# trevorcampbell/bayesian-coresets

Measured on AMD Instinct MI355X. Metric: greedy coreset iterations/sec (N=10000000, d=512), higher is better.
Workload: dtype f32 scan + f64 state

## Files before the change

bayesian-coresets_amd/csrc/api.hip:

```cpp
#include <stdio.h>
#include <string.h>
#include <algorithm>
#include <cmath>
#include "bcx_internal.h"
#include "dev_util.h"

static thread_local std::string g_create_err;
namespace {
void bounce_acquire(int device);
void bounce_release(int device);
}

extern "C" const char* bcx_version(void) { return "bcx 0.1 gfx950"; }

extern "C" const char* bcx_last_error(const bcx_solver* s) { return s ? s->err.c_str() : g_create_err.c_str(); }

template <typename T> static hipError_t dev_alloc(T** p, size_t count, bool zero = true) {
  *p = nullptr;
  if (count == 0) count = 1;
  hipError_t e = hipMalloc((void**)p, count * sizeof(T));
  if (e != hipSuccess) return e;
  if (zero) e = hipMemset(*p, 0, count * sizeof(T));
  return e;
}

static int round_up(int x, int m) { return (x + m - 1) / m * m; }

static void free_all(bcx_solver* s) {
  void* ptrs[] = {s->An, s->A64, s->norms, s->chunk_sums, s->staging, s->st, s->b, s->bn, s->xw, s->q64, s->qst,
                  s->tmp, s->partials, s->rec_local, s->act_idx, s->act_w, s->act_rows, s->act_norm, s->gram,
                  s->hinv, s->hinv_lo, s->cvec, s->plist, s->ppos, s->nn_x, s->nn_z, s->nn_wv, s->nn_tmp, s->nn_flag, s->nn_wbak, s->nn_xr, s->tr_sel, s->tr_err,
                  s->tr_status};
  for (void* p : ptrs)
    if (p) (void)hipFree(p);
  for (size_t w = 0; w < s->peer_mbox.size(); ++w)
    if (s->peer_mbox[w] && s->peer_mbox[w] != s->mbox) (void)hipIpcCloseMemHandle(s->peer_mbox[w]);
  void* xptrs[] = {s->mbox, s->peer_tab, s->xseq, s->xprobe, s->rec_gather, s->grid_counter, s->fin_part, s->gram_work, s->warm_buf,
                   s->Aq, s->scr_sb, s->scr_partials, s->scr_stat, s->A4, s->s4_sb, s->s4_list, s->s4_counts, s->s4_head};
  for (void* p : xptrs)
    if (p) (void)hipFree(p);
  for (auto& ev : s->prof_events) { (void)hipEventDestroy(ev.first); (void)hipEventDestroy(ev.second); }
}

extern "C" int bcx_create(const bcx_config* cfg, bcx_solver** out) {
  if (!cfg || !out) { g_create_err = "bcx_create: null argument"; return BCX_ERR_ARG; }
  *out = nullptr;
  if (cfg->alg < BCX_ALG_GIGA || cfg->alg > BCX_ALG_OMP || cfg->d < 1 || cfg->n_local < 0 ||
      cfg->world_size < 1 || cfg->rank < 0 || cfg->rank >= cfg->world_size ||
      (cfg->store_dtype != BCX_F32 && cfg->store_dtype != BCX_F64 && cfg->store_dtype != BCX_F16)) {
    g_create_err = "bcx_create: invalid configuration";
    return BCX_ERR_ARG;
  }
  const int maxd = BCX_MAX_D;
  if (cfg->d > maxd) { g_create_err = "bcx_create: d exceeds the supported row length (" + std::to_string(maxd) + ")"; return BCX_ERR_ARG; }
  if (cfg->n_local >= (int64_t)0x7fffffff) { g_create_err = "bcx_create: n_local must be < 2^31 per shard"; return BCX_ERR_ARG; }
  if (cfg->row_offset % BCX_CHUNK_ROWS != 0) {
    g_create_err = "bcx_create: row_offset must be a multiple of the chunk size (1024 rows)";
    return BCX_ERR_ARG;
  }
  bcx_solver* s = new bcx_solver();
  s->cfg = *cfg;
  if (s->cfg.refresh_every == 0) s->cfg.refresh_every = 64;
  if (const char* e = bcx_dev_env("BCX_SCREEN8")) s->scr_enabled = atoi(e) != 0;
  if (const char* e = bcx_dev_env("BCX_SCREEN4_SEGCAP")) { const int v = atoi(e); if (v >= 1 && v <= BCX_S4_SEG_CAP) s->s4_seg_cap = v; }
  if (const char* e = bcx_dev_env("BCX_SCREEN4")) s->s4_enabled = atoi(e) != 0;
  hipError_t e = hipSetDevice(cfg->device);
  if (e != hipSuccess) { g_create_err = std::string("hipSetDevice: ") + hipGetErrorString(e); delete s; return BCX_ERR_HIP; }
  const int d = cfg->d;
  const int64_t n = cfg->n_local;
  s->elem = cfg->store_dtype == BCX_F32 ? 4 : (cfg->store_dtype == BCX_F16 ? 2 : 8);
  s->qelem = cfg->store_dtype == BCX_F64 ? 8 : 4;
  s->ld = round_up(d, 16 / s->elem);
  s->ld64 = round_up(d, 2);
  s->n_chunks = (n + BCX_CHUNK_ROWS - 1) / BCX_CHUNK_ROWS;
  bool ok = true;
  auto chk = [&](hipError_t r) { if (r != hipSuccess && ok) { ok = false; g_create_err = std::string("hipMalloc: ") + hipGetErrorString(r); } };
  chk(dev_alloc((char**)&s->An, (size_t)n * s->ld * s->elem));
  if (cfg->keep_exact_rows && cfg->store_dtype != BCX_F64) chk(dev_alloc(&s->A64, (size_t)n * s->ld64));
  chk(dev_alloc(&s->norms, (size_t)n));
  chk(dev_alloc(&s->chunk_sums, (size_t)s->n_chunks * (d + 1)));
  chk(dev_alloc(&s->st, 1));
  chk(dev_alloc(&s->b, (size_t)d));
  chk(dev_alloc(&s->bn, (size_t)d));
  chk(dev_alloc(&s->xw, (size_t)d));
  chk(dev_alloc(&s->q64, (size_t)2 * s->ld64));
  chk(dev_alloc((char**)&s->qst, (size_t)2 * s->ld * s->qelem));
  chk(dev_alloc(&s->tmp, (size_t)20 * d));
  s->n_partials = 0;
  chk(dev_alloc((char**)&s->partials, (size_t)bcx_scan_grid(s) * BCX_PARTIAL_BYTES));
  chk(dev_alloc(&s->rec_local, (size_t)(d + BCX_REC_HDR)));
  if (!ok) { free_all(s); delete s; return BCX_ERR_NOMEM; }
  bounce_acquire(cfg->device);
  *out = s;
  return BCX_OK;
}

extern "C" int bcx_destroy(bcx_solver* s) {
  if (!s) return BCX_OK;
  (void)hipSetDevice(s->cfg.device);
  (void)hipDeviceSynchronize();
  free_all(s);
  bounce_release(s->cfg.device);
  delete s;
  return BCX_OK;
}

extern "C" int bcx_set_stream(bcx_solver* s, void* hip_stream) {
  if (!s) return BCX_ERR_ARG;
  s->stream = (hipStream_t)hip_stream;
  return BCX_OK;
}

static int read_state(bcx_solver* s, DevState* h);

#include <mutex>
#include <thread>
namespace {
constexpr size_t kBounceBytes = (size_t)32 << 20;
constexpr int kMaxDevices = 64;
struct Bounce {
  std::mutex mu;
  void* buf[2] = {nullptr, nullptr};
  int users = 0;
};
Bounce g_bounce[kMaxDevices];
Bounce& bounce_of(int device) { return g_bounce[(device >= 0 && device < kMaxDevices) ? device : 0]; }
void bounce_acquire(int device) {
  Bounce& b = bounce_of(device);
  std::lock_guard<std::mutex> lock(b.mu);
  b.users += 1;
}
void bounce_release(int device) {
  Bounce& b = bounce_of(device);
  std::lock_guard<std::mutex> lock(b.mu);
  if (--b.users <= 0) {
    b.users = 0;
    for (int i = 0; i < 2; ++i)
      if (b.buf[i]) { (void)hipHostFree(b.buf[i]); b.buf[i] = nullptr; }
  }
}

void copy_rows_mt(char* dst, size_t dpitch, const char* src, size_t spitch, size_t width, int64_t rows) {
  const size_t bytes = (size_t)rows * width;
  int nt = (int)std::min<size_t>(8, bytes / ((size_t)2 << 20));
  const unsigned hw = std::thread::hardware_concurrency();
  if (hw && (unsigned)nt > hw) nt = (int)hw;
  auto work = [=](int64_t r0, int64_t r1) {
    if (dpitch == width && spitch == width) { memcpy(dst + (size_t)r0 * width, src + (size_t)r0 * width, (size_t)(r1 - r0) * width); return; }
    for (int64_t r = r0; r < r1; ++r) memcpy(dst + (size_t)r * dpitch, src + (size_t)r * spitch, width);
  };
  if (nt <= 1) { work(0, rows); return; }
  std::vector<std::thread> th;
  const int64_t per = (rows + nt - 1) / nt;
  for (int t = 1; t < nt; ++t) {
    const int64_t r0 = std::min<int64_t>(rows, t * per), r1 = std::min<int64_t>(rows, (t + 1) * per);
    if (r0 < r1) th.emplace_back(work, r0, r1);
  }
  work(0, std::min<int64_t>(rows, per));
  for (auto& t : th) t.join();
}
}

static int upload_host_rows(bcx_solver* s, void* dst_dev, size_t dpitch, const void* src, size_t spitch, size_t width,
                            int64_t rows) {
  if (rows <= 0) return BCX_OK;
  Bounce& g_b = bounce_of(s->cfg.device);
  std::lock_guard<std::mutex> lock(g_b.mu);
  for (int i = 0; i < 2; ++i)
    if (!g_b.buf[i]) BCX_HIP(hipHostMalloc(&g_b.buf[i], kBounceBytes, hipHostMallocPortable));
  if (width > kBounceBytes) { s->err = "bcx_load_rows: a row exceeds the upload buffer"; return BCX_ERR_ARG; }
  hipEvent_t done[2] = {nullptr, nullptr};
  bool busy[2] = {false, false};
  for (int i = 0; i < 2; ++i) {
    const hipError_t ee = hipEventCreateWithFlags(&done[i], hipEventDisableTiming);
    if (ee != hipSuccess) {
      if (i == 1) (void)hipEventDestroy(done[0]);
      s->err = std::string("upload: ") + hipGetErrorString(ee);
      return BCX_ERR_HIP;
    }
  }
  const int64_t rows_per = std::max<int64_t>(1, (int64_t)(kBounceBytes / width));
  int which = 0;
  int rc = BCX_OK;
  for (int64_t r = 0; r < rows && rc == BCX_OK; r += rows_per, which ^= 1) {
    const int64_t m = std::min(rows_per, rows - r);
    if (busy[which]) {
      if (hipEventSynchronize(done[which]) != hipSuccess) { s->err = "upload: event wait failed"; rc = BCX_ERR_HIP; break; }
      busy[which] = false;
    }
    copy_rows_mt((char*)g_b.buf[which], width, (const char*)src + (size_t)r * spitch, spitch, width, m);
    hipError_t e = hipMemcpy2DAsync((char*)dst_dev + (size_t)r * dpitch, dpitch, g_b.buf[which], width, width, (size_t)m,
                                    hipMemcpyHostToDevice, s->stream);
    if (e == hipSuccess) e = hipEventRecord(done[which], s->stream);
    if (e != hipSuccess) { s->err = std::string("upload: ") + hipGetErrorString(e); rc = BCX_ERR_HIP; break; }
    busy[which] = true;
  }
  for (int i = 0; i < 2; ++i) {
    if (busy[i]) (void)hipEventSynchronize(done[i]);
    (void)hipEventDestroy(done[i]);
  }
  return rc;
}


static int load_rows(bcx_solver* s, const void* src, int32_t src_is_device, int32_t src_dtype, int64_t row_begin,
                     int64_t rows, int64_t ld, int32_t flags);

extern "C" int bcx_load_rows(bcx_solver* s, const void* src, int32_t src_is_device, int32_t src_dtype,
                             int64_t row_begin, int64_t rows, int64_t ld) {
  return load_rows(s, src, src_is_device, src_dtype, row_begin, rows, ld, 0);
}

extern "C" int bcx_load_rows_flags(bcx_solver* s, const void* src, int32_t src_is_device, int32_t src_dtype,
                                   int64_t row_begin, int64_t rows, int64_t ld, int32_t flags) {
  if (flags & ~BCX_LOAD_CENTER_ROWS) { if (s) s->err = "bcx_load_rows_flags: unknown flag"; return BCX_ERR_ARG; }
  return load_rows(s, src, src_is_device, src_dtype, row_begin, rows, ld, flags);
}

static int load_rows(bcx_solver* s, const void* src, int32_t src_is_device, int32_t src_dtype, int64_t row_begin,
                     int64_t rows, int64_t ld, int32_t flags) {
  if (!s || (!src && rows > 0)) return BCX_ERR_ARG;
  const int center = (flags & BCX_LOAD_CENTER_ROWS) ? 1 : 0;
  const int d = s->cfg.d;
  if (rows == 0) return BCX_OK;
  if (row_begin < 0 || rows < 0 || row_begin + rows > s->cfg.n_local || ld < d ||
      (src_dtype != BCX_F32 && src_dtype != BCX_F64)) {
    s->err = "bcx_load_rows: bad range, leading dimension or dtype";
    return BCX_ERR_ARG;
  }
  if (row_begin % BCX_CHUNK_ROWS != 0 || (rows % BCX_CHUNK_ROWS != 0 && row_begin + rows != s->cfg.n_local)) {
    s->err = "bcx_load_rows: pieces must start and end on 1024-row chunk boundaries (except the last)";
    return BCX_ERR_ARG;
  }
  BCX_HIP(hipSetDevice(s->cfg.device));
  if (row_begin == 0) {
    if (s->finalized || s->rows_loaded > 0) {
      DevState h;
      int rc0 = read_state(s, &h);
      if (rc0 != BCX_OK) return rc0;
      h.zero_row = 0; h.k = 0; h.np = 0; h.hvalid = 1; h.omp_ill = 0; h.limit = 0; h.active = 0; h.halt = HALT_NONE;
      BCX_HIP(hipMemcpy(s->st, &h, sizeof h, hipMemcpyHostToDevice));
      s->finalized = false;
    }
    s->rows_loaded = 0;
  }
  const size_t esz = src_dtype == BCX_F64 ? 8 : 4;
  if (src_is_device) {
    int rc = bcx_launch_ingest(s, src, src_dtype, ld, row_begin, rows, center);
    if (rc != BCX_OK) return rc;
  } else if (s->A64 && src_dtype == BCX_F64) {
    double* dst = s->A64 + (size_t)row_begin * s->ld64;
    int rc = upload_host_rows(s, dst, (size_t)s->ld64 * 8, src, (size_t)ld * 8, (size_t)d * 8, rows);
    if (rc != BCX_OK) return rc;
    rc = bcx_launch_ingest(s, dst, BCX_F64, s->ld64, row_begin, rows, center);
    if (rc != BCX_OK) return rc;
  } else {
    const int64_t piece = std::max<int64_t>(BCX_CHUNK_ROWS,
                                            ((int64_t)(256u << 20) / (int64_t)(d * esz)) / BCX_CHUNK_ROWS * BCX_CHUNK_ROWS);
    const size_t need = (size_t)std::min(piece, rows) * d * esz;
    if (s->staging_bytes < need) {
      if (s->staging) BCX_HIP(hipFree(s->staging));
      s->staging = nullptr; s->staging_bytes = 0;
      BCX_HIP(hipMalloc(&s->staging, need));
      s->staging_bytes = need;
    }
    for (int64_t r = 0; r < rows; r += piece) {
      const int64_t m = std::min(piece, rows - r);
      int rc = upload_host_rows(s, s->staging, (size_t)d * esz, (const char*)src + (size_t)r * ld * esz, (size_t)ld * esz,
                                (size_t)d * esz, m);
      if (rc != BCX_OK) return rc;
      rc = bcx_launch_ingest(s, s->staging, src_dtype, d, row_begin + r, m, center);
      if (rc != BCX_OK) return rc;
      BCX_HIP(hipStreamSynchronize(s->stream));
    }
  }
  s->rows_loaded += rows;
  s->scr_valid = false;
  s->s4_valid = false;
  return BCX_OK;
}

extern "C" int bcx_chunk_sums(bcx_solver* s, const void** dev_ptr, int64_t* n_chunks, int64_t* chunk_rows) {
  if (!s) return BCX_ERR_ARG;
  if (dev_ptr) *dev_ptr = s->chunk_sums;
  if (n_chunks) *n_chunks = s->n_chunks;
  if (chunk_rows) *chunk_rows = BCX_CHUNK_ROWS;
  return BCX_OK;
}

extern "C" int bcx_export_chunk_sums(bcx_solver* s, void* dst_dev, int64_t cap_chunks) {
  if (!s || !dst_dev || cap_chunks < s->n_chunks) return BCX_ERR_ARG;
  BCX_HIP(hipMemcpyAsync(dst_dev, s->chunk_sums, (size_t)s->n_chunks * (s->cfg.d + 1) * 8, hipMemcpyDeviceToDevice,
                         s->stream));
  return BCX_OK;
}

static int read_state(bcx_solver* s, DevState* h) {
  BCX_HIP(hipStreamSynchronize(s->stream));
  BCX_HIP(hipMemcpy(h, s->st, sizeof(DevState), hipMemcpyDeviceToHost));
  return BCX_OK;
}

extern "C" int bcx_finalize(bcx_solver* s, const double* b_host, const void* gathered_sums_dev, int64_t n_gathered) {
  if (!s) return BCX_ERR_ARG;
  BCX_HIP(hipSetDevice(s->cfg.device));
  if (s->rows_loaded < s->cfg.n_local) { s->err = "bcx_finalize: not all rows were loaded"; return BCX_ERR_STATE; }
  if (b_host) BCX_HIP(hipMemcpyAsync(s->b, b_host, (size_t)s->cfg.d * 8, hipMemcpyHostToDevice, s->stream));
  int rc = bcx_launch_finalize(s, b_host != nullptr, (const double*)gathered_sums_dev, n_gathered);
  if (rc != BCX_OK) return rc;
  DevState h;
  rc = read_state(s, &h);
  if (rc != BCX_OK) return rc;
  if (h.zero_row != 0) {
    char buf[128];
    snprintf(buf, sizeof buf, "A must not have any 0 columns (local row %d has zero norm)", h.zero_row - 1);
    s->err = buf;
    return BCX_ERR_ZERO_ROW;
  }
  if (s->cfg.alg == BCX_ALG_GIGA && h.bnorm == 0.0) { s->err = "norm of b must be > 0"; return BCX_ERR_ZERO_B; }
  s->finalized = true;
  return BCX_OK;
}

template <typename T> static int grow(bcx_solver* s, T** p, size_t old_count, size_t new_count) {
  T* q = nullptr;
  BCX_HIP(dev_alloc(&q, new_count));
  if (*p && old_count) BCX_HIP(hipMemcpy(q, *p, old_count * sizeof(T), hipMemcpyDeviceToDevice));
  if (*p) BCX_HIP(hipFree(*p));
  *p = q;
  return BCX_OK;
}

static int ensure_slots(bcx_solver* s, int64_t need) {
  if (need <= s->cap) return BCX_OK;
  int64_t ncap = std::max<int64_t>(need, std::max<int64_t>(256, s->cap * 2));
  const size_t d = (size_t)s->cfg.d;
  int rc;
  if ((rc = grow(s, &s->act_idx, (size_t)s->cap, (size_t)ncap))) return rc;
  if ((rc = grow(s, &s->act_w, (size_t)s->cap, (size_t)ncap))) return rc;
  if ((rc = grow(s, &s->act_norm, (size_t)s->cap, (size_t)ncap))) return rc;
  if ((rc = grow(s, &s->act_rows, (size_t)s->cap * d, (size_t)ncap * d))) return rc;
  s->cap = ncap;
  return BCX_OK;
}

int bcx_ensure_gram(bcx_solver* s, int64_t need) {
  if (need <= s->gram_cap) return BCX_OK;
  const int64_t ncap = std::max<int64_t>((need + 63) / 64 * 64, std::max<int64_t>(256, s->gram_cap * 2));
  const size_t oc = (size_t)s->gram_cap, nc = (size_t)ncap;
  double* g2 = nullptr; double* h2 = nullptr; double* l2 = nullptr;
  BCX_HIP(dev_alloc(&g2, nc * nc));
  BCX_HIP(dev_alloc(&h2, nc * nc));
  BCX_HIP(dev_alloc(&l2, nc * nc));
  if (oc) {
    BCX_HIP(hipMemcpy2D(g2, nc * 8, s->gram, oc * 8, oc * 8, oc, hipMemcpyDeviceToDevice));
    BCX_HIP(hipMemcpy2D(h2, nc * 8, s->hinv, oc * 8, oc * 8, oc, hipMemcpyDeviceToDevice));
    BCX_HIP(hipMemcpy2D(l2, nc * 8, s->hinv_lo, oc * 8, oc * 8, oc, hipMemcpyDeviceToDevice));
    BCX_HIP(hipFree(s->gram));
    BCX_HIP(hipFree(s->hinv));
    BCX_HIP(hipFree(s->hinv_lo));
  }
  s->gram = g2; s->hinv = h2; s->hinv_lo = l2;
  int rc;
  if ((rc = grow(s, &s->cvec, oc, nc))) return rc;
  if ((rc = grow(s, &s->plist, oc, nc))) return rc;
  if ((rc = grow(s, &s->ppos, oc, nc))) return rc;
  if ((rc = grow(s, &s->nn_x, oc, nc))) return rc;
  if ((rc = grow(s, &s->nn_z, 0, nc))) return rc;
  if ((rc = grow(s, &s->nn_wv, 0, nc))) return rc;
  if ((rc = grow(s, &s->nn_tmp, 0, 16 * nc))) return rc;
  if ((rc = grow(s, &s->nn_flag, 0, nc))) return rc;
  if ((rc = grow(s, &s->nn_wbak, 0, nc))) return rc;
  if ((rc = grow(s, &s->nn_xr, 0, 2 * nc))) return rc;
  s->gram_cap = ncap;
  return BCX_OK;
}

static int ensure_trace(bcx_solver* s, int64_t need) {
  if (need <= s->trace_cap) return BCX_OK;
  int64_t ncap = std::max<int64_t>(need, 1024);
  int rc;
  if ((rc = grow(s, &s->tr_sel, 0, (size_t)ncap))) return rc;
  if ((rc = grow(s, &s->tr_err, 0, (size_t)ncap))) return rc;
  if ((rc = grow(s, &s->tr_status, 0, (size_t)ncap))) return rc;
  s->trace_cap = ncap;
  return BCX_OK;
}

extern "C" int bcx_build_begin(bcx_solver* s, int64_t itrs, double tol, int32_t* skip) {
  if (!s || !skip) return BCX_ERR_ARG;
  if (!s->finalized) { s->err = "bcx_build_begin: call bcx_finalize first"; return BCX_ERR_STATE; }
  BCX_HIP(hipSetDevice(s->cfg.device));
  *skip = 0;
  DevState h;
  int rc = read_state(s, &h);
  if (rc != BCX_OK) return rc;
  if (h.limit || s->cfg.n_global == 0 || itrs <= 0) { *skip = 1; return BCX_OK; }
  s->k_ub = h.k;
  if ((rc = ensure_slots(s, (int64_t)h.k + itrs))) return rc;
  if (s->cfg.alg == BCX_ALG_OMP) {
    if ((rc = bcx_ensure_gram(s, (int64_t)h.k + itrs))) return rc;
    if (!s->grid_counter && dev_alloc(&s->grid_counter, 32 ) != hipSuccess) { s->err = "grid counter allocation failed"; return BCX_ERR_NOMEM; }
    BCX_HIP(hipMemsetAsync(s->grid_counter, 0, 2 * sizeof(unsigned long long), s->stream));
    s->grid_epoch = 0;
    s->grid_dirty = false;
  }
  if ((rc = ensure_trace(s, itrs))) return rc;
  return bcx_launch_begin(s, itrs, tol);
}

static int prof_begin(bcx_solver* s) {
  if (!s->profile) return BCX_OK;
  s->prof_now = (s->prof_tick++ % s->prof_every) == 0;
  if (!s->prof_now) return BCX_OK;
  if (s->prof_used == s->prof_events.size()) {
    hipEvent_t a, b;
    BCX_HIP(hipEventCreate(&a));
    BCX_HIP(hipEventCreate(&b));
    s->prof_events.emplace_back(a, b);
  }
  BCX_HIP(hipEventRecord(s->prof_events[s->prof_used].first, s->stream));
  return BCX_OK;
}
static int prof_end(bcx_solver* s) {
  if (!s->profile || !s->prof_now) return BCX_OK;
  BCX_HIP(hipEventRecord(s->prof_events[s->prof_used].second, s->stream));
  s->prof_used++;
  return BCX_OK;
}

static int step_scan(bcx_solver* s, void* send_dev, int exact, bool with_tail) {
  if (!s->finalized) { s->err = "solver not finalized"; return BCX_ERR_STATE; }
  double* send = send_dev ? (double*)send_dev : s->rec_local;
  int rc;
  if (exact && (rc = bcx_launch_resume_exact(s))) return rc;
  if ((rc = prof_begin(s))) return rc;
  if ((rc = bcx_launch_scan(s, exact))) return rc;
  if ((rc = prof_end(s))) return rc;
  if (with_tail) return bcx_launch_tail(s, exact);
  return bcx_launch_resolve(s, send, exact);
}

static int front_scan(bcx_solver* s, int exact, bool tier, bool four) {
  int rc;
  if (exact && (rc = bcx_launch_resume_exact(s))) return rc;
  if ((rc = prof_begin(s))) return rc;
  if ((rc = (tier && !exact) ? (four ? bcx_launch_screen4(s) : bcx_launch_screen(s)) : bcx_launch_scan(s, exact))) return rc;
  return prof_end(s);
}

extern "C" int bcx_step_scan(bcx_solver* s, void* send_dev) { if (s) s->scr_batch = false; return s ? step_scan(s, send_dev, 0, false) : BCX_ERR_ARG; }
extern "C" int bcx_step_scan_exact(bcx_solver* s, void* send_dev) { if (s) s->scr_batch = false; return s ? step_scan(s, send_dev, 1, false) : BCX_ERR_ARG; }

extern "C" int bcx_step_apply(bcx_solver* s, const void* recv_dev) {
  if (!s) return BCX_ERR_ARG;
  return bcx_launch_apply(s, recv_dev ? (const double*)recv_dev : s->rec_local);
}

static int enqueue_one(bcx_solver* s, int exact, bool tier, bool four = false) {
  if (!s->finalized) { s->err = "solver not finalized"; return BCX_ERR_STATE; }
  int rc;
  if (s->cfg.world_size != 1) {
    if (!s->exchange_ready) {
      s->err = "bcx_build_enqueue on a row shard needs bcx_exchange_attach (or drive bcx_step_scan / bcx_step_apply)";
      return BCX_ERR_ARG;
    }
    if ((rc = front_scan(s, exact, tier, false))) return rc;
    return bcx_launch_tail_exchange(s, exact);
  }
  if ((rc = front_scan(s, exact, tier, four))) return rc;
  if (s->cfg.alg == BCX_ALG_OMP) {
    rc = bcx_launch_omp_fused(s, exact);
    if (rc != 1) return rc;
    if ((rc = bcx_launch_resolve(s, s->rec_local, exact))) return rc;
    return bcx_launch_apply(s, s->rec_local);
  }
  return bcx_launch_tail(s, exact);
}

static int enqueue_many(bcx_solver* s, int64_t itrs) {
  int rc = bcx_screen_build(s);
  if (rc != BCX_OK) return rc;
  const bool tier = bcx_screen_on(s) && s->scr_valid;
  if (tier && (rc = bcx_screen4_build(s))) return rc;
  const bool tier4 = tier && bcx_screen4_on(s) && s->s4_valid;
  s->scr_batch = false;
  for (int64_t i = 0; i < itrs; ++i) {
    s->scr_batch = tier;
    const bool four = tier4 && s->s4_warm == 0;
    rc = enqueue_one(s, 0, tier, four);
    if (rc != BCX_OK) return rc;
    if (tier && s->s4_warm > 0) s->s4_warm -= 1;
  }
  return BCX_OK;
}

extern "C" int bcx_build_enqueue(bcx_solver* s, int64_t itrs) {
  if (!s) return BCX_ERR_ARG;
  if (!s->finalized) { s->err = "solver not finalized"; return BCX_ERR_STATE; }
  return enqueue_many(s, itrs);
}

extern "C" int bcx_build_enqueue_exact(bcx_solver* s) {
  if (!s) return BCX_ERR_ARG;
  if (!s->finalized) { s->err = "solver not finalized"; return BCX_ERR_STATE; }
  s->scr_batch = false;
  return enqueue_one(s, 1, false);
}

static int mailbox_alloc(bcx_solver* s) {
  if (s->mbox) return BCX_OK;
  const int world = s->cfg.world_size;
  const size_t bytes = bcx_mailbox_slot_offset(world) + 2 * (size_t)world * (s->cfg.d + BCX_REC_HDR) * sizeof(double);
  hipError_t e = hipExtMallocWithFlags(&s->mbox, bytes, hipDeviceMallocFinegrained);
  if (e != hipSuccess) {
    (void)hipGetLastError();
    s->mbox = nullptr;
    s->err = std::string("peer mailbox: fine-grained allocation failed: ") + hipGetErrorString(e);
    return BCX_ERR_HIP;
  }
  s->mbox_bytes = bytes;
  BCX_HIP(hipMemset(s->mbox, 0, bytes));
  BCX_HIP(hipDeviceSynchronize());
  return BCX_OK;
}

extern "C" int bcx_exchange_export(bcx_solver* s, void* handle_out, int32_t handle_bytes) {
  if (!s || !handle_out) return BCX_ERR_ARG;
  if (handle_bytes < (int32_t)sizeof(hipIpcMemHandle_t)) { s->err = "bcx_exchange_export: handle buffer too small"; return BCX_ERR_ARG; }
  if ((size_t)s->cfg.d * sizeof(double) > 144 * 1024) {
    s->err = "peer mailbox: rows of more than 18432 values exchange their records through the all-gather";
    return BCX_ERR_ARG;
  }
  BCX_HIP(hipSetDevice(s->cfg.device));
  int rc = mailbox_alloc(s);
  if (rc != BCX_OK) return rc;
  hipIpcMemHandle_t h;
  BCX_HIP(hipIpcGetMemHandle(&h, s->mbox));
  memset(handle_out, 0, handle_bytes);
  memcpy(handle_out, &h, sizeof(h));
  return BCX_OK;
}

extern "C" int bcx_exchange_attach(bcx_solver* s, const void* handles, int32_t handle_bytes, double timeout_s) {
  if (!s || !handles) return BCX_ERR_ARG;
  if (s->exchange_ready) return BCX_OK;
  if (!s->mbox) { s->err = "bcx_exchange_attach: call bcx_exchange_export first"; return BCX_ERR_STATE; }
  if (handle_bytes < (int32_t)sizeof(hipIpcMemHandle_t)) return BCX_ERR_ARG;
  BCX_HIP(hipSetDevice(s->cfg.device));
  const int world = s->cfg.world_size;
  if (world > BCX_APPLY_THREADS) { s->err = "peer mailbox supports at most 256 shards"; return BCX_ERR_ARG; }
  s->peer_mbox.assign(world, nullptr);
  for (int w = 0; w < world; ++w) {
    if (w == s->cfg.rank) { s->peer_mbox[w] = s->mbox; continue; }
    hipIpcMemHandle_t h;
    memcpy(&h, (const char*)handles + (size_t)w * handle_bytes, sizeof(h));
    hipError_t e = hipIpcOpenMemHandle(&s->peer_mbox[w], h, hipIpcMemLazyEnablePeerAccess);
    if (e != hipSuccess) {
      (void)hipGetLastError();
      s->peer_mbox[w] = nullptr;
      s->err = "peer mailbox: cannot map shard " + std::to_string(w) + ": " + hipGetErrorString(e);
      for (int v = 0; v < w; ++v)
        if (v != s->cfg.rank && s->peer_mbox[v]) { (void)hipIpcCloseMemHandle(s->peer_mbox[v]); s->peer_mbox[v] = nullptr; }
      s->peer_mbox.clear();
      return BCX_ERR_HIP;
    }
  }
  hipError_t e;
  if ((e = dev_alloc(&s->peer_tab, (size_t)world)) != hipSuccess || (e = dev_alloc(&s->xseq, 8)) != hipSuccess ||
      (e = dev_alloc(&s->xprobe, 1)) != hipSuccess ||
      (e = dev_alloc(&s->rec_gather, (size_t)world * (s->cfg.d + BCX_REC_HDR))) != hipSuccess) {
    s->err = std::string("peer mailbox: ") + hipGetErrorString(e);
    return BCX_ERR_NOMEM;
  }
  BCX_HIP(hipMemcpy(s->peer_tab, s->peer_mbox.data(), (size_t)world * sizeof(void*), hipMemcpyHostToDevice));
  if (timeout_s > 0.0) s->exchange_timeout_s = timeout_s;
  s->exchange_ready = true;
  return BCX_OK;
}

extern "C" int bcx_exchange_probe(bcx_solver* s, int32_t* result) {
  if (!s || !result) return BCX_ERR_ARG;
  if (!s->exchange_ready) { s->err = "bcx_exchange_probe: no peer mailbox attached"; return BCX_ERR_STATE; }
  BCX_HIP(hipSetDevice(s->cfg.device));
  int rc = bcx_launch_exchange_probe(s);
  if (rc != BCX_OK) return rc;
  BCX_HIP(hipStreamSynchronize(s->stream));
  BCX_HIP(hipMemcpy(result, s->xprobe, sizeof(int32_t), hipMemcpyDeviceToHost));
  return BCX_OK;
}

extern "C" int bcx_exchange_set_timeout(bcx_solver* s, double timeout_s) {
  if (!s || !(timeout_s > 0.0)) return BCX_ERR_ARG;
  s->exchange_timeout_s = timeout_s;
  return BCX_OK;
}

extern "C" int bcx_exchange_stats(bcx_solver* s, int64_t* n, double* wait_us_mean, double* wait_us_max, double* total_us_mean,
                                  double* total_us_max, int32_t reset) {
  if (!s) return BCX_ERR_ARG;
  unsigned long long h[5] = {0, 0, 0, 0, 0};
  if (s->xseq) {
    BCX_HIP(hipSetDevice(s->cfg.device));
    BCX_HIP(hipStreamSynchronize(s->stream));
    BCX_HIP(hipMemcpy(h, s->xseq + 1, sizeof h, hipMemcpyDeviceToHost));
    if (reset) BCX_HIP(hipMemset(s->xseq + 1, 0, sizeof h));
  }
  const double per = h[0] ? 1.0 / (double)h[0] : 0.0, us = 1.0 / 100.0;
  if (n) *n = (int64_t)h[0];
  if (wait_us_mean) *wait_us_mean = (double)h[1] * per * us;
  if (wait_us_max) *wait_us_max = (double)h[2] * us;
  if (total_us_mean) *total_us_mean = (double)h[3] * per * us;
  if (total_us_max) *total_us_max = (double)h[4] * us;
  return BCX_OK;
}

extern "C" int bcx_exchange_disable(bcx_solver* s) {
  if (!s) return BCX_ERR_ARG;
  s->exchange_ready = false;
  return BCX_OK;
}

extern "C" int bcx_build_poll(bcx_solver* s, int64_t* n_done, int32_t* need_exact, int32_t* limit) {
  if (!s) return BCX_ERR_ARG;
  DevState h;
  int rc = read_state(s, &h);
  if (rc != BCX_OK) return rc;
  while (h.halt == HALT_NEED_EXACT && s->scr_batch && s->scr_stat) {
    unsigned long long st8[SCR_WORDS];
    BCX_HIP(hipMemcpy(st8, s->scr_stat, sizeof st8, hipMemcpyDeviceToHost));
    if (!st8[SCR_ARMED]) break;
    if (st8[SCR4_LAST] != 0 && st8[SCR4_LAST] == st8[SCR_ITERS]) {
      s->s4_halts += 1;
      for (int i = 3; i > 0; --i) s->s4_ovf_at[i] = s->s4_ovf_at[i - 1];
      s->s4_ovf_at[0] = st8[SCR4_ITERS];
      s->s4_redos += 1;
      if (s->s4_halts >= 4 && s->s4_ovf_at[0] - s->s4_ovf_at[3] < 256 && !s->s4_dropped) { s->s4_dropped = 1; s->s4_drops += 1; }
    } else {
      s->scr_halts += 1;
      for (int i = 3; i > 0; --i) s->scr_ovf_at[i] = s->scr_ovf_at[i - 1];
      s->scr_ovf_at[0] = st8[SCR_ITERS];
      if (s->scr_halts >= 4 && s->scr_ovf_at[0] - s->scr_ovf_at[3] < 256) s->scr_dropped = 1;
    }
    if (s->s4_warm < 1) s->s4_warm = 1;
    if ((rc = bcx_launch_resume_store(s))) return rc;
    if ((rc = enqueue_one(s, 0, false))) return rc;
    const int64_t rest = h.itrs - h.it - 1;
    if (rest > 0 && (rc = enqueue_many(s, rest))) return rc;
    else if (rest <= 0) s->scr_batch = false;
    if ((rc = read_state(s, &h))) return rc;
  }
  if (h.halt == HALT_GRID_TIMEOUT) { s->err = "OMP step: grid barrier timed out"; return BCX_ERR_STATE; }
  if (h.halt == HALT_EXCHANGE_TIMEOUT) {
    unsigned long long late[2] = {0, 0};
    std::string who;
    if (s->xseq && hipMemcpy(late, s->xseq + 6, sizeof late, hipMemcpyDeviceToHost) == hipSuccess) {
      for (int r = 0; r < s->cfg.world_size && r < 64; ++r)
        if (late[0] >> r & 1ull) who += (who.empty() ? "" : ", ") + std::to_string(r);
      (void)hipMemset(s->xseq + 6, 0, sizeof late);
    } else (void)hipGetLastError();
    s->err = "peer mailbox: rank " + std::to_string(s->cfg.rank) + " got no record from rank(s) " + (who.empty() ? "?" : who) +
             " within " + std::to_string(s->exchange_timeout_s) + " s (exchange #" + std::to_string(late[1]) + ")";
    return BCX_ERR_EXCHANGE;
  }
  if (n_done) *n_done = h.it;
  if (need_exact) *need_exact = (h.halt == HALT_NEED_EXACT);
  if (limit) *limit = h.limit;
  if (s->profile) {
    const bool on8 = bcx_screen_on(s) && s->scr_valid;
    const double min_ms = (double)s->cfg.n_local * s->cfg.d * (on8 ? ((bcx_screen4_on(s) && s->s4_valid) ? 0.5 : 1.0) : (double)s->elem) / 12.0e9;
    for (size_t i = 0; i < s->prof_used; ++i) {
      float ms = 0.f;
      if (hipEventElapsedTime(&ms, s->prof_events[i].first, s->prof_events[i].second) != hipSuccess) continue;
      if ((double)ms >= min_ms) { s->prof_ms += ms; s->prof_launches += 1; }
    }
    s->prof_used = 0;
  }
  return BCX_OK;
}

extern "C" int bcx_build_trace(bcx_solver* s, int64_t* sel, double* err, int32_t* status, int64_t cap, int64_t* n_out) {
  if (!s) return BCX_ERR_ARG;
  DevState h;
  int rc = read_state(s, &h);
  if (rc != BCX_OK) return rc;
  const int64_t n = std::min<int64_t>(h.it, cap);
  if (n > 0) {
    if (sel) BCX_HIP(hipMemcpy(sel, s->tr_sel, (size_t)n * 8, hipMemcpyDeviceToHost));
    if (err) BCX_HIP(hipMemcpy(err, s->tr_err, (size_t)n * 8, hipMemcpyDeviceToHost));
    if (status) BCX_HIP(hipMemcpy(status, s->tr_status, (size_t)n * 4, hipMemcpyDeviceToHost));
  }
  if (n_out) *n_out = n;
  return BCX_OK;
}

extern "C" int bcx_active_count(bcx_solver* s, int64_t* k) {
  if (!s || !k) return BCX_ERR_ARG;
  DevState h;
  int rc = read_state(s, &h);
  if (rc != BCX_OK) return rc;
  *k = h.k;
  return BCX_OK;
}

extern "C" int bcx_get_weights(bcx_solver* s, int64_t* idx, double* w, int64_t cap, int64_t* k) {
  if (!s || !k) return BCX_ERR_ARG;
  DevState h;
  int rc = read_state(s, &h);
  if (rc != BCX_OK) return rc;
  const int64_t n = std::min<int64_t>(h.k, cap);
  if (n > 0) {
    if (idx) BCX_HIP(hipMemcpy(idx, s->act_idx, (size_t)n * 8, hipMemcpyDeviceToHost));
    if (w) BCX_HIP(hipMemcpy(w, s->act_w, (size_t)n * 8, hipMemcpyDeviceToHost));
  }
  *k = h.k;
  return BCX_OK;
}

extern "C" int bcx_error(bcx_solver* s, double* err) {
  if (!s || !err) return BCX_ERR_ARG;
  if (!s->finalized) { s->err = "solver not finalized"; return BCX_ERR_STATE; }
  int rc = bcx_launch_error_refresh(s);
  if (rc != BCX_OK) return rc;
  DevState h;
  if ((rc = read_state(s, &h))) return rc;
  *err = h.err;
  return BCX_OK;
}

extern "C" int bcx_reached_numeric_limit(bcx_solver* s, int32_t* limit) {
  if (!s || !limit) return BCX_ERR_ARG;
  DevState h;
  int rc = read_state(s, &h);
  if (rc != BCX_OK) return rc;
  *limit = h.limit;
  return BCX_OK;
}

extern "C" int bcx_reset(bcx_solver* s) {
  if (!s) return BCX_ERR_ARG;
  if (!s->finalized) return BCX_OK;
  DevState h;
  int rc = read_state(s, &h);
  if (rc != BCX_OK) return rc;
  h.k = 0; h.np = 0; h.hvalid = 1; h.omp_ill = 0; h.limit = 0; h.retried = 0; h.active = 0; h.halt = HALT_NONE; h.since_refresh = 0; h.exact_mode = 0;
  h.err = h.bnorm; h.nw = 1.0; h.it = 0; h.itrs = 0;
  BCX_HIP(hipMemcpy(s->st, &h, sizeof h, hipMemcpyHostToDevice));
  BCX_HIP(hipMemset(s->xw, 0, (size_t)s->cfg.d * 8));
  if (s->scr_dropped == 1) s->scr_dropped = 0;
  s->scr_halts = 0;
  for (int i = 0; i < 4; ++i) s->scr_ovf_at[i] = 0;
  if (s->s4_dropped == 1) s->s4_dropped = 0;
  s->s4_halts = 0;
  for (int i = 0; i < 4; ++i) s->s4_ovf_at[i] = 0;
  s->s4_warm = 2;
  return bcx_launch_error_refresh(s);
}

extern "C" int bcx_set_check_monotone(bcx_solver* s, int32_t on) {
  if (!s) return BCX_ERR_ARG;
  BCX_HIP(hipSetDevice(s->cfg.device));
  DevState h;
  int rc = read_state(s, &h);
  if (rc != BCX_OK) return rc;
  h.no_monotone = on ? 0 : 1;
  BCX_HIP(hipMemcpy(s->st, &h, sizeof h, hipMemcpyHostToDevice));
  return BCX_OK;
}

extern "C" int bcx_optimize(bcx_solver* s, double tol, int32_t* accepted) {
  if (!s || !accepted) return BCX_ERR_ARG;
  if (!s->finalized) { s->err = "solver not finalized"; return BCX_ERR_STATE; }
  DevState h;
  int rc = read_state(s, &h);
  if (rc != BCX_OK) return rc;
  if ((rc = ensure_slots(s, std::max<int64_t>(h.k, 1)))) return rc;
  if ((rc = bcx_ensure_gram(s, std::max<int64_t>(h.k, 1)))) return rc;
  if ((rc = bcx_launch_optimize(s, tol))) return rc;
  DevState h2;
  if ((rc = read_state(s, &h2))) return rc;
  if (h2.halt == HALT_GRID_TIMEOUT) { s->err = "optimize: grid barrier timed out"; return BCX_ERR_STATE; }
  *accepted = h2.limit ? 0 : 1;
  return BCX_OK;
}

extern "C" int bcx_get_vector(bcx_solver* s, int32_t which, double* out) {
  if (!s || !out) return BCX_ERR_ARG;
  const double* src = nullptr;
  switch (which) {
    case 0: src = s->b; break;
    case 1: src = s->xw; break;
    case 2: src = s->q64; break;
    case 3: src = s->q64 + s->ld64; break;
    default: return BCX_ERR_ARG;
  }
  BCX_HIP(hipStreamSynchronize(s->stream));
  BCX_HIP(hipMemcpy(out, src, (size_t)s->cfg.d * 8, hipMemcpyDeviceToHost));
  return BCX_OK;
}

extern "C" int bcx_get_norms(bcx_solver* s, int64_t begin, int64_t count, double* out) {
  if (!s || !out || begin < 0 || begin + count > s->cfg.n_local) return BCX_ERR_ARG;
  BCX_HIP(hipStreamSynchronize(s->stream));
  BCX_HIP(hipMemcpy(out, s->norms + begin, (size_t)count * 8, hipMemcpyDeviceToHost));
  return BCX_OK;
}

extern "C" int bcx_get_stored_rows(bcx_solver* s, int64_t begin, int64_t count, void* out, int32_t* ld_out) {
  if (!s || begin < 0 || count < 0 || begin + count > s->cfg.n_local) return BCX_ERR_ARG;
  if (ld_out) *ld_out = s->ld;
  if (count == 0) return BCX_OK;
  if (!out) return BCX_ERR_ARG;
  BCX_HIP(hipSetDevice(s->cfg.device));
  BCX_HIP(hipStreamSynchronize(s->stream));
  BCX_HIP(hipMemcpy(out, (const char*)s->An + (size_t)begin * s->ld * s->elem, (size_t)count * s->ld * s->elem, hipMemcpyDeviceToHost));
  return BCX_OK;
}

extern "C" int bcx_time_scan(bcx_solver* s, int32_t reps, int32_t exact, double* ms_per_launch, double* bytes_per_launch) {
  if (!s || reps < 1) return BCX_ERR_ARG;
  if (!s->finalized) { s->err = "solver not finalized"; return BCX_ERR_STATE; }
  BCX_HIP(hipSetDevice(s->cfg.device));
  DevState h;
  int rc = read_state(s, &h);
  if (rc != BCX_OK) return rc;
  DevState forced = h;
  forced.active = 1;
  BCX_HIP(hipMemcpy(s->st, &forced, sizeof forced, hipMemcpyHostToDevice));
  hipEvent_t e0, e1;
  BCX_HIP(hipEventCreate(&e0));
  BCX_HIP(hipEventCreate(&e1));
  for (int i = 0; i < 3 && rc == BCX_OK; ++i) rc = bcx_launch_scan(s, exact);
  if (rc == BCX_OK) (void)hipEventRecord(e0, s->stream);
  for (int i = 0; i < reps && rc == BCX_OK; ++i) rc = bcx_launch_scan(s, exact);
  if (rc != BCX_OK) {
    (void)hipEventDestroy(e0); (void)hipEventDestroy(e1);
    (void)hipMemcpy(s->st, &h, sizeof h, hipMemcpyHostToDevice);
    return rc;
  }
  BCX_HIP(hipEventRecord(e1, s->stream));
  BCX_HIP(hipEventSynchronize(e1));
  float ms = 0.f;
  BCX_HIP(hipEventElapsedTime(&ms, e0, e1));
  BCX_HIP(hipEventDestroy(e0));
  BCX_HIP(hipEventDestroy(e1));
  BCX_HIP(hipMemcpy(s->st, &h, sizeof h, hipMemcpyHostToDevice));
  if (ms_per_launch) *ms_per_launch = (double)ms / reps;
  const bool raw64 = exact && s->cfg.store_dtype != BCX_F64 && s->A64;
  if (bytes_per_launch) *bytes_per_launch = (double)s->cfg.n_local * s->cfg.d * (raw64 ? 8.0 : (double)s->elem);
  return BCX_OK;
}

extern "C" int bcx_argmax_correlation(bcx_solver* s, const double* query_host, int64_t* idx, double* score) {
  if (!s || !query_host || !idx || !score) return BCX_ERR_ARG;
  if (!s->finalized) { s->err = "solver not finalized"; return BCX_ERR_STATE; }
  if (s->cfg.alg == BCX_ALG_GIGA) { s->err = "bcx_argmax_correlation needs a single-query solver (FW/OMP)"; return BCX_ERR_ARG; }
  BCX_HIP(hipSetDevice(s->cfg.device));
  const int d = s->cfg.d;
  DevState h;
  int rc = read_state(s, &h);
  if (rc != BCX_OK) return rc;
  std::vector<double> q64((size_t)s->ld64, 0.0);
  double qmax = 0.0;
  for (int j = 0; j < d; ++j) { q64[j] = query_host[j]; qmax = std::fmax(qmax, std::fabs(query_host[j])); }
  const bool scalable = qmax > 0.0 && qmax < INFINITY;
  const int E0 = scalable ? std::ilogb(qmax) : 0;
  double qn = 0.0;
  for (int j = 0; j < d; ++j) { const double t = std::ldexp(query_host[j], -E0); qn += t * t; }
  qn = std::sqrt(qn);
  int E = 0;
  BCX_HIP(hipMemcpy(s->q64, q64.data(), (size_t)s->ld64 * 8, hipMemcpyHostToDevice));
  if (s->cfg.store_dtype == BCX_F64) {
    std::vector<double> qs((size_t)s->ld, 0.0);
    for (int j = 0; j < d; ++j) qs[j] = query_host[j];
    BCX_HIP(hipMemcpy(s->qst, qs.data(), (size_t)s->ld * 8, hipMemcpyHostToDevice));
    qn = std::ldexp(qn, E0);
  } else {
    const int E1 = (scalable && qn > 0.0 && qn < INFINITY) ? std::ilogb(qn) : 0;
    E = E0 + E1;
    std::vector<float> qs((size_t)s->ld, 0.f);
    for (int j = 0; j < d; ++j) qs[j] = (float)std::ldexp(query_host[j], -E);
    BCX_HIP(hipMemcpy(s->qst, qs.data(), (size_t)s->ld * 4, hipMemcpyHostToDevice));
    qn = std::ldexp(qn, -E1);
  }
  DevState forced = h;
  forced.active = 1; forced.exact_mode = 0; forced.qscale = qn; forced.qexp = E;
  double rec[BCX_REC_HDR];
  for (int attempt = 0; attempt < 2; ++attempt) {
    forced.exact_mode = attempt;
    BCX_HIP(hipMemcpy(s->st, &forced, sizeof forced, hipMemcpyHostToDevice));
    if ((rc = bcx_launch_scan(s, attempt))) return rc;
    if ((rc = bcx_launch_resolve(s, s->rec_local, attempt))) return rc;
    BCX_HIP(hipStreamSynchronize(s->stream));
    BCX_HIP(hipMemcpy(rec, s->rec_local, sizeof rec, hipMemcpyDeviceToHost));
    if (rec[3] != BCX_REC_OVERFLOW) break;
  }
  BCX_HIP(hipMemcpy(s->st, &h, sizeof h, hipMemcpyHostToDevice));
  if (rec[3] != BCX_REC_VALID) { s->err = "no rows to scan"; return BCX_ERR_STATE; }
  *idx = (int64_t)rec[1];
  *score = rec[0];
  return BCX_OK;
}

extern "C" int bcx_stats(bcx_solver* s, int64_t* exact_fallbacks, int64_t* candidates, int64_t* resolves) {
  if (!s) return BCX_ERR_ARG;
  DevState h;
  int rc = read_state(s, &h);
  if (rc != BCX_OK) return rc;
  if (exact_fallbacks) *exact_fallbacks = h.n_exact;
  if (candidates) *candidates = h.n_cand;
  if (resolves) *resolves = h.n_resolved;
  return BCX_OK;
}

extern "C" int bcx_screen_stats(bcx_solver* s, int64_t* out8) {
  if (!s || !out8) return BCX_ERR_ARG;
  unsigned long long st8[SCR_WORDS] = {0, 0, 0, 0, 0, 0, 0, 0};
  if (s->scr_stat) {
    BCX_HIP(hipSetDevice(s->cfg.device));
    BCX_HIP(hipStreamSynchronize(s->stream));
    BCX_HIP(hipMemcpy(st8, s->scr_stat, sizeof st8, hipMemcpyDeviceToHost));
  }
  const bool possible = s->scr_enabled && s->cfg.store_dtype != BCX_F64 && s->cfg.d <= 4096 && s->cfg.n_local > 0;
  out8[0] = bcx_screen_on(s) ? 1 : 0;
  out8[1] = (int64_t)st8[SCR_ITERS];
  out8[2] = (int64_t)st8[SCR_SURVIVORS];
  out8[3] = (int64_t)st8[SCR_OVERFLOWS];
  out8[4] = (int64_t)st8[SCR_REDOS];
  out8[5] = !possible ? 3 : s->scr_dropped;
  out8[6] = s->Aq ? (int64_t)s->scr_cap_rows * (s->ld8 + 8) + (int64_t)BCX_MAX_PARTIALS * BCX_PARTIAL_BYTES + SCR_WORDS * 8 : 0;
  out8[7] = (int64_t)(s->scr_build_ms * 1e3f);
  return BCX_OK;
}

extern "C" int bcx_screen4_stats(bcx_solver* s, int64_t* out8) {
  if (!s || !out8) return BCX_ERR_ARG;
  unsigned long long st8[SCR_WORDS];
  for (auto& w : st8) w = 0;
  if (s->scr_stat) {
    BCX_HIP(hipSetDevice(s->cfg.device));
    BCX_HIP(hipStreamSynchronize(s->stream));
    BCX_HIP(hipMemcpy(st8, s->scr_stat, sizeof st8, hipMemcpyDeviceToHost));
  }
  const bool possible = s->s4_enabled && s->scr_enabled && s->cfg.store_dtype != BCX_F64 && s->cfg.d <= 4096 && s->cfg.n_local > 0 &&
                        s->cfg.alg != BCX_ALG_GIGA && s->cfg.world_size == 1;
  if (st8[SCR4_PENDING] && s->s4_counts && s->s4_n_seg > 0) {
    std::vector<int32_t> cnt((size_t)s->s4_n_seg);
    BCX_HIP(hipMemcpy(cnt.data(), s->s4_counts, cnt.size() * 4, hipMemcpyDeviceToHost));
    for (int32_t c : cnt) { st8[SCR4_LISTED] += (unsigned long long)std::min<int32_t>(c, s->s4_seg_cap); st8[SCR4_OVERFLOWS] += c > s->s4_seg_cap; }
  }
  out8[0] = bcx_screen4_on(s) ? 1 : 0;
  out8[1] = (int64_t)st8[SCR4_ITERS];
  out8[2] = (int64_t)st8[SCR4_LISTED];
  out8[3] = (int64_t)st8[SCR4_OVERFLOWS];
  out8[4] = s->s4_redos;
  out8[5] = !possible ? 3 : s->s4_dropped;
  out8[6] = s->A4 ? (int64_t)s->s4_cap_rows * (s->ld4 + 8) + (int64_t)BCX_MAX_PARTIALS * (BCX_S4_SEG_CAP + 1) * 4 : 0;
  out8[7] = s->s4_drops;
  return BCX_OK;
}

extern "C" int bcx_screen_read(bcx_solver* s, int64_t begin, int64_t count, void* codes, float* scales, float* bounds, int32_t* ld8_out) {
  if (!s || begin < 0 || count < 0 || begin + count > s->cfg.n_local) return BCX_ERR_ARG;
  if (!s->finalized) { s->err = "solver not finalized"; return BCX_ERR_STATE; }
  BCX_HIP(hipSetDevice(s->cfg.device));
  int rc = bcx_screen_build(s);
  if (rc != BCX_OK) return rc;
  if (!bcx_screen_on(s) || !s->scr_valid) { s->err = "bcx_screen_read: the 8-bit tier is not in use"; return BCX_ERR_STATE; }
  BCX_HIP(hipStreamSynchronize(s->stream));
  if (ld8_out) *ld8_out = s->ld8;
  if (count == 0) return BCX_OK;
  if (codes) BCX_HIP(hipMemcpy(codes, (const char*)s->Aq + (size_t)begin * s->ld8, (size_t)count * s->ld8, hipMemcpyDeviceToHost));
  std::vector<float> sb((size_t)count * 2);
  BCX_HIP(hipMemcpy(sb.data(), (const char*)s->scr_sb + (size_t)begin * 8, (size_t)count * 8, hipMemcpyDeviceToHost));
  for (int64_t i = 0; i < count; ++i) {
    if (scales) scales[i] = sb[2 * i];
    if (bounds) bounds[i] = sb[2 * i + 1];
  }
  return BCX_OK;
}

extern "C" int bcx_omp_stats(bcx_solver* s, int64_t* out4) {
  if (!s || !out4) return BCX_ERR_ARG;
  DevState h;
  int rc = read_state(s, &h);
  if (rc != BCX_OK) return rc;
  for (int i = 0; i < 4; ++i) out4[i] = h.n_omp[i];
  out4[2] += s->opt_fallbacks;
  return BCX_OK;
}

extern "C" int bcx_profile_scan(bcx_solver* s, int32_t on) {
  if (!s) return BCX_ERR_ARG;
  s->profile = on != 0;
  s->prof_every = on > 1 ? on : 1;
  s->prof_tick = 0;
  s->prof_ms = 0.0;
  s->prof_launches = 0;
  s->prof_used = 0;
  return BCX_OK;
}

extern "C" int bcx_profile_read(bcx_solver* s, double* scan_ms_total, int64_t* scan_launches) {
  if (!s) return BCX_ERR_ARG;
  if (scan_ms_total) *scan_ms_total = s->prof_ms;
  if (scan_launches) *scan_launches = s->prof_launches;
  return BCX_OK;
}

extern "C" int bcx_debug_stamps(bcx_solver* s, long long* out32) {
  DevState h;
  int rc = read_state(s, &h);
  if (rc != BCX_OK) return rc;
  for (int i = 0; i < 32; ++i) out32[i] = h.dbg_t[i];
  return BCX_OK;
}

extern "C" int bcx_debug_wbak(bcx_solver* s, double* out, int32_t count) {
  if (!s || !s->nn_wbak || count > s->gram_cap) return BCX_ERR_ARG;
  BCX_HIP(hipDeviceSynchronize());
  BCX_HIP(hipMemcpy(out, s->nn_wbak, (size_t)count * sizeof(double), hipMemcpyDeviceToHost));
  return BCX_OK;
}
```

bayesian-coresets_amd/csrc/bcx_internal.h:

```cpp
#pragma once
#include <hip/hip_runtime.h>
#include <stdint.h>
#include <string>
#include <utility>
#include <vector>
#include "../../include/bcx.h"

#define BCX_CHUNK_ROWS 1024
#define BCX_MAX_CAND 64
#define BCX_REC_HDR 4
#define BCX_REC_VALID 1.0
#define BCX_REC_OVERFLOW 2.0
#define BCX_MAX_D BCX_MAX_ROW_LENGTH
#define BCX_SCAN_THREADS 256
#define BCX_APPLY_THREADS 256

enum { HALT_NONE = 0, HALT_DONE = 1, HALT_LIMIT = 2, HALT_NEED_EXACT = 3, HALT_EXCHANGE_TIMEOUT = 4, HALT_GRID_TIMEOUT = 5 };
enum { OMP_IDLE = 0, OMP_DONE = 1, OMP_FAST_TRY = 2, OMP_FAST_ACCEPT = 3, OMP_GENERAL = 4,
       OMP_OPT_FALLBACK = 5 };

struct PartialView {
  double *U1, *U2, *U3, *L;
  int32_t *i1, *i2;
};
#define BCX_PARTIAL_BYTES 40
#define BCX_MAX_PARTIALS 2048
#define BCX_SCREEN_MAX_SURV 256
enum { SCR_ARMED = 0,
       SCR_ITERS = 1,
       SCR_SURVIVORS = 2,
       SCR_OVERFLOWS = 3,
       SCR_REDOS = 4,
       SCR4_ITERS = 5,
       SCR4_LISTED = 6,
       SCR4_OVERFLOWS = 7,
       SCR4_LAST = 8,
       SCR4_PENDING = 9,
       SCR_WORDS = 10 };
#define BCX_S4_SEG_CAP 1024
#define BCX_S4_SENTINELS 64
static inline __host__ __device__ PartialView partial_view(void* base, int n) {
  PartialView v;
  v.U1 = (double*)base; v.U2 = v.U1 + n; v.U3 = v.U2 + n; v.L = v.U3 + n;
  v.i1 = (int32_t*)(v.L + n); v.i2 = v.i1 + n;
  return v;
}

struct Mailbox {
  void* const* peers;
  unsigned long long* seq;
  int32_t* probe;
  unsigned long long* stat;
  int world, rank, recw;
  unsigned off_slots;
  long long timeout_ticks;
};

static inline unsigned bcx_mailbox_slot_offset(int world) { return (unsigned)((2u * world * 8u + 255u) / 256u * 256u); }

struct DevState {
  int64_t itrs;
  int64_t it;
  int32_t active;
  int32_t halt;
  int32_t retried;
  int32_t limit;
  int32_t k;
  int32_t since_refresh;
  int32_t exact_mode;
  int32_t zero_row;
  int32_t no_monotone;
  int32_t np;
  int32_t hvalid;
  int32_t hlo_valid;
  int32_t omp_mode;
  int32_t omp_slot, omp_fresh, omp_checked, omp_p;
  int32_t omp_ill;
  int64_t omp_f;
  double omp_nf, omp_gff, omp_cf, omp_t, omp_inv;
  double tol;
  double err;
  double nw;
  double bnorm;
  double sigma;
  int64_t n_exact;
  int64_t n_cand;
  int64_t n_resolved;
  int64_t n_omp[4];
  double qscale;
  int32_t qexp;
  int32_t qexp_pad;
  long long dbg_t[32];
};

struct bcx_solver {
  bcx_config cfg;
  hipStream_t stream = nullptr;
  std::string err;
  int ld = 0;
  int elem = 4;
  int qelem = 4;
  int ld64 = 0;
  void* An = nullptr;
  double* A64 = nullptr;
  double* norms = nullptr;
  double* chunk_sums = nullptr;
  int64_t n_chunks = 0;
  void* staging = nullptr;
  size_t staging_bytes = 0;
  DevState* st = nullptr;
  double* b = nullptr;
  double* bn = nullptr;
  double* xw = nullptr;
  double* q64 = nullptr;
  void* qst = nullptr;
  double* tmp = nullptr;
  void* partials = nullptr;
  int n_partials = 0;
  double* rec_local = nullptr;
  double* fin_part = nullptr;
  int64_t fin_cap = 0;
  void* mbox = nullptr;
  size_t mbox_bytes = 0;
  std::vector<void*> peer_mbox;
  void** peer_tab = nullptr;
  unsigned long long* xseq = nullptr;
  int32_t* xprobe = nullptr;
  double* rec_gather = nullptr;
  bool exchange_ready = false;
  double exchange_timeout_s = 20.0;
  int64_t cap = 0;
  int64_t* act_idx = nullptr;
  double* act_w = nullptr;
  double* act_rows = nullptr;
  double* act_norm = nullptr;
  double* gram = nullptr;
  double* hinv = nullptr;
  double* hinv_lo = nullptr;
  double* cvec = nullptr;
  int32_t* plist = nullptr;
  int32_t* ppos = nullptr;
  double* nn_x = nullptr;
  double* nn_z = nullptr;
  double* nn_wv = nullptr;
  double* nn_tmp = nullptr;
  int32_t* nn_flag = nullptr;
  double* nn_wbak = nullptr;
  double* nn_xr = nullptr;
  int64_t gram_cap = 0;
  double* gram_work = nullptr;
  size_t gram_work_bytes = 0;
  void* warm_buf = nullptr;
  size_t warm_bytes = 0;
  int64_t opt_warm = 0, opt_warm_failed = 0;
  int64_t k_ub = 0;
  unsigned long long* grid_counter = nullptr;
  uint64_t grid_epoch = 0;
  int64_t opt_fallbacks = 0;
  bool grid_dirty = false;
  size_t omp_lds_allowed = 0;
  int64_t trace_cap = 0;
  int64_t* tr_sel = nullptr;
  double* tr_err = nullptr;
  int32_t* tr_status = nullptr;
  bool finalized = false;
  int64_t rows_loaded = 0;
  void* Aq = nullptr;
  void* scr_sb = nullptr;
  void* scr_partials = nullptr;
  unsigned long long* scr_stat = nullptr;
  int ld8 = 0;
  int64_t scr_cap_rows = 0;
  bool scr_enabled = true;
  int scr_dropped = 0;
  bool scr_valid = false;
  bool scr_batch = false;
  float scr_build_ms = 0.f;
  uint64_t scr_ovf_at[4] = {0, 0, 0, 0};
  int64_t scr_halts = 0;
  int scr_n_in = 0;
  void* A4 = nullptr;
  void* s4_sb = nullptr;
  void* s4_list = nullptr;
  void* s4_counts = nullptr;
  void* s4_head = nullptr;
  int ld4 = 0;
  int s4_n_seg = 0;
  int s4_seg_cap = BCX_S4_SEG_CAP;
  int64_t s4_cap_rows = 0;
  bool s4_enabled = true;
  int s4_dropped = 0;
  bool s4_valid = false;
  int s4_warm = 2;
  uint64_t s4_ovf_at[4] = {0, 0, 0, 0};
  int64_t s4_halts = 0;
  int64_t s4_redos = 0, s4_drops = 0;
  bool profile = false;
  bool prof_now = false;
  int prof_every = 1;
  int64_t prof_tick = 0;
  double prof_ms = 0.0;
  int64_t prof_launches = 0;
  std::vector<std::pair<hipEvent_t, hipEvent_t>> prof_events;
  size_t prof_used = 0;
};

int bcx_launch_ingest(bcx_solver* s, const void* src, int src_dtype, int64_t ld_src, int64_t row_begin, int64_t rows,
                      int center);
int bcx_launch_finalize(bcx_solver* s, int have_b, const double* gathered, int64_t n_gathered);
int bcx_launch_scan(bcx_solver* s, int exact);
int bcx_launch_resolve(bcx_solver* s, double* send_dev, int exact);
int bcx_launch_begin(bcx_solver* s, int64_t itrs, double tol);
int bcx_launch_apply(bcx_solver* s, const double* recv_dev);
int bcx_launch_tail(bcx_solver* s, int exact);
int bcx_launch_omp_fused(bcx_solver* s, int exact);
int bcx_launch_tail_exchange(bcx_solver* s, int exact);
int bcx_launch_exchange_probe(bcx_solver* s);
Mailbox bcx_mailbox(const bcx_solver* s);
int bcx_launch_resume_exact(bcx_solver* s);
int bcx_launch_error_refresh(bcx_solver* s);
int bcx_launch_optimize(bcx_solver* s, double tol);
int64_t bcx_gram_rows_scratch_bytes(int k, int d);
int bcx_gram_rows(hipStream_t st, const double* rows, int k, int d, int64_t ld, double* G, int64_t ldg, double* work);
unsigned long long bcx_gram_sk_epoch_now();
int bcx_gram_sk_timed_out(hipStream_t st, const double* work, unsigned long long since);
int bcx_scan_grid(const bcx_solver* s);
bool bcx_screen_on(const bcx_solver* s);
int bcx_screen_build(bcx_solver* s);
int bcx_launch_screen(bcx_solver* s);
int bcx_launch_resume_store(bcx_solver* s);
int bcx_launch_refine(bcx_solver* s, int n_in);
bool bcx_screen4_on(const bcx_solver* s);
int bcx_screen4_build(bcx_solver* s);
int bcx_launch_screen4(bcx_solver* s);
void bcx_project_set_error(const std::string& msg);
const double* proj_tables();

#ifdef BCX_TIMING
#define BCX_STAMP(st, i) do { if (threadIdx.x == 0) (st)->dbg_t[i] = wall_clock64(); } while (0)
#else
#define BCX_STAMP(st, i) do {} while (0)
#endif

#define BCX_HIP(call)                                                        \
  do {                                                                       \
    hipError_t _e = (call);                                                  \
    if (_e != hipSuccess) {                                                  \
      s->err = std::string(#call) + ": " + hipGetErrorString(_e);            \
      return BCX_ERR_HIP;                                                    \
    }                                                                        \
  } while (0)
```

bayesian-coresets_amd/csrc/screen4.hip:

```cpp
#include <float.h>
#include "screen_core.h"

#define BCX_S4_CLIP 0.8
#define BCX_S4_QMAX 1911.0
#define BCX_THRESH_THREADS 1024

struct Front4Head { float Lg, qstep, eA, eB; };

template <int CTRL> __device__ __forceinline__ int dpp_mov_i(int v) { return __builtin_amdgcn_update_dpp(0, v, CTRL, 0xf, 0xf, false); }
template <int G> __device__ __forceinline__ int group_allsum_i32(int v) {
  if (G >= 2) v += dpp_mov_i<0xB1>(v);
  if (G >= 4) v += dpp_mov_i<0x4E>(v);
  if (G >= 8) v += dpp_mov_i<0x141>(v);
  if (G >= 16) v += dpp_mov_i<0x140>(v);
  if (G >= 32) { const v2u r = __builtin_amdgcn_permlane16_swap((unsigned)v, (unsigned)v, false, false); const unsigned x = r.x, y = r.y; v = (int)(x + y); }
  if (G >= 64) { const v2u r = __builtin_amdgcn_permlane32_swap((unsigned)v, (unsigned)v, false, false); const unsigned x = r.x, y = r.y; v = (int)(x + y); }
  return v;
}

static __device__ __forceinline__ float round_up_f32(double v) {
  float f = (float)v;
  if ((double)f < v) f = nextafterf(f, INFINITY);
  return f;
}

struct Thresh4Args {
  PartialView in;
  int n_in;
  const unsigned char* Aq;
  const float2* sb;
  const float* q;
  const DevState* st;
  unsigned long long* stat;
  unsigned* head;
  const int* counts;
  int n_seg;
  int seg_cap;
  int64_t n;
  int ld8, d, nw4;
  float kacc, err_coef;
};

__global__ __launch_bounds__(BCX_THRESH_THREADS) void thresh4_kernel(Thresh4Args a) {
  if (!a.st->active) return;
  __shared__ double scratch[BCX_SCRATCH];
  const int tid = threadIdx.x, lane = tid & 63, wave = tid >> 6;
  constexpr int NW = BCX_THRESH_THREADS / 64;
  constexpr int PT = 2 * BCX_MAX_PARTIALS / BCX_THRESH_THREADS;
  double cu[PT];
  int ci[PT];
#pragma unroll
  for (int t = 0; t < PT; ++t) {
    const int c = wave + NW * (lane + 64 * t);
    const int p = c >> 1;
    const bool ok = p < a.n_in;
    const double u = ok ? ((c & 1) ? a.in.U2[p] : a.in.U1[p]) : -INFINITY;
    const int i = ok ? ((c & 1) ? a.in.i2[p] : a.in.i1[p]) : -1;
    const bool use = u > -INFINITY && i >= 0 && (int64_t)i < a.n;
    cu[t] = use ? u : -INFINITY; ci[t] = use ? i : -1;
  }
  double m = 0.0;
  for (int j = tid; j < a.d; j += BCX_THRESH_THREADS) {
    const double v = fabs((double)a.q[j]);
    m = fmax(m, v == v ? v : INFINITY);
  }
  m = block_allmax(m, scratch);
  float step = (float)(m / BCX_S4_QMAX);
  const bool qok = m < INFINITY && step >= FLT_MIN;
  if (!qok) step = 0.0f;
  constexpr int SPW = BCX_S4_SENTINELS / NW;
  int rows[SPW];
#pragma unroll
  for (int r = 0; r < SPW; ++r) {
    double best = -INFINITY;
    int bt = -1, bi = -1;
#pragma unroll
    for (int t = 0; t < PT; ++t) if (cu[t] > best) { best = cu[t]; bt = t; bi = ci[t]; }
    const double wm = wave_allmax(best);
    const unsigned long long bal = __ballot(bt >= 0 && best == wm);
    const int src = bal ? __ffsll((long long)bal) - 1 : 0;
    const int row = __shfl(bi, src, BCX_WAVE);
    rows[r] = bal ? row : -1;
#pragma unroll
    for (int t = 0; t < PT; ++t) if (bal && lane == src && t == bt) cu[t] = -INFINITY;
  }
  double acc[SPW];
#pragma unroll
  for (int r = 0; r < SPW; ++r) acc[r] = 0.0;
  const int nw8 = a.ld8 / 4;
  const unsigned* A8 = (const unsigned*)a.Aq;
  for (int w = lane; w < nw8; w += 64) {
    unsigned cw[SPW];
#pragma unroll
    for (int r = 0; r < SPW; ++r) cw[r] = A8[(int64_t)(rows[r] < 0 ? 0 : rows[r]) * nw8 + w];
    double qv[4];
#pragma unroll
    for (int k = 0; k < 4; ++k) { const int j = 4 * w + k; const float t = a.q[j < a.d ? j : 0]; qv[k] = j < a.d ? (double)t : 0.0; }
#pragma unroll
    for (int r = 0; r < SPW; ++r)
#pragma unroll
      for (int k = 0; k < 4; ++k) acc[r] = fma((double)((int)((cw[r] >> (8 * k)) & 0xffu) - 128), qv[k], acc[r]);
  }
  double err2[3] = {0.0, 0.0, 0.0};
  if (a.stat[SCR4_PENDING])
    for (int p = tid; p < a.n_seg; p += BCX_THRESH_THREADS) {
      const int c = a.counts[p];
      err2[1] += (double)(c > a.seg_cap ? a.seg_cap : c);
      err2[2] += c > a.seg_cap ? 1.0 : 0.0;
    }
  for (int w = tid; w < a.nw4; w += BCX_THRESH_THREADS) {
    unsigned p0 = 0, p1 = 0, p2 = 0;
#pragma unroll
    for (int k = 0; k < 8; ++k) {
      const int j = 8 * w + k;
      int x = 0;
      if (j < a.d && qok) {
        const double v = (double)a.q[j];
        double c = rint(v / (double)step);
        c = c > BCX_S4_QMAX ? BCX_S4_QMAX : (c < -BCX_S4_QMAX ? -BCX_S4_QMAX : c);
        x = (int)c;
        const double r = v - c * (double)step;
        err2[0] = fma(r, r, err2[0]);
      }
      const int l = ((x + 8) & 15) - 8;
      const int x1 = (x - l) >> 4;
      const int h1 = ((x1 + 8) & 15) - 8;
      const int h2 = (x1 - h1) >> 4;
      p0 |= (unsigned)(l & 15) << (4 * k); p1 |= (unsigned)(h1 & 15) << (4 * k); p2 |= (unsigned)(h2 & 15) << (4 * k);
    }
    a.head[4 + w] = p0; a.head[4 + a.nw4 + w] = p1; a.head[4 + 2 * a.nw4 + w] = p2;
  }
  block_allsum<3>(err2, scratch);
  const double qerr = sqrt(err2[0]) * (1.0 + 9.5367431640625e-07);
  const float qscale = (float)a.st->qscale;
  float lmax = -INFINITY;
#pragma unroll
  for (int r = 0; r < SPW; ++r) {
    const double tot = wave_allsum(acc[r]);
    const float2 sb = a.sb[rows[r] < 0 ? 0 : rows[r]];
    const float s0 = (float)((double)sb.x * tot);
    float U, L;
    screen_interval(s0, sb.x, sb.y, a.kacc, a.err_coef, qscale, U, L);
    if (rows[r] >= 0) lmax = fmaxf(lmax, L);
  }
  const double lg = block_allmax((double)lmax, scratch);
  if (tid == 0) {
    const double qs = (double)qscale;
    Front4Head h;
    h.Lg = qok ? (float)lg : -INFINITY;
    h.qstep = step;
    h.eA = round_up_f32((qs * 1.000002 + qerr) * 1.000004);
    h.eB = round_up_f32(((double)a.err_coef * qs + 1.001 * qerr) * 1.000004 + 1e-37);
    *(Front4Head*)a.head = h;
    a.stat[SCR4_LAST] = a.stat[SCR_ITERS] + 1ull;
    a.stat[SCR4_ITERS] += 1ull;
    a.stat[SCR4_LISTED] += (unsigned long long)err2[1];
    a.stat[SCR4_OVERFLOWS] += (unsigned long long)err2[2];
    a.stat[SCR4_PENDING] = 1ull;
  }
}

struct Front4Args {
  const uint4* A4;
  const float2* sb;
  const unsigned* head;
  const DevState* st;
  int* list;
  int* counts;
  int64_t n;
  int ldv, nw4, seg_cap;
};

template <int G, int CH, int UR>
__global__ __launch_bounds__(BCX_SCAN_THREADS) void front4_kernel(Front4Args a) {
  if (!a.st->active) return;
  constexpr int RPW = 64 / G;
  constexpr int WAVES = BCX_SCREEN_WAVES;
  constexpr int RPB = WAVES * RPW * UR;
  const int lane = threadIdx.x & 63, wave = threadIdx.x >> 6;
  const int sub = lane % G, rsub = lane / G;
  const Front4Head h = *(const Front4Head*)a.head;
  const unsigned* planes = a.head + 4;
  int qp[CH][4][3];
  int voff[CH];
#pragma unroll
  for (int c = 0; c < CH; ++c) {
    const int v = c * G + sub;
    const bool ok = v < a.ldv;
    voff[c] = ok ? v : 0;
#pragma unroll
    for (int k = 0; k < 4; ++k)
#pragma unroll
      for (int p = 0; p < 3; ++p) {
        const unsigned w = planes[p * a.nw4 + 4 * voff[c] + k];
        qp[c][k][p] = ok ? (int)w : 0;
      }
  }
  const int b = blockIdx.x * WAVES + wave;
  int* seg = a.list + (size_t)b * BCX_S4_SEG_CAP;
  int cnt = 0;
  const int64_t n = a.n;
  const int64_t stride = (int64_t)gridDim.x * RPB;
  for (int64_t r0 = (int64_t)blockIdx.x * RPB; r0 < n; r0 += stride) {
    uint4 x[UR][CH];
    float2 sbv[UR];
#pragma unroll
    for (int u = 0; u < UR; ++u) {
      const int64_t rw = r0 + (int64_t)(u * WAVES + wave) * RPW + rsub;
      const int64_t rc = rw < n ? rw : n - 1;
      const uint4* p = a.A4 + rc * a.ldv;
#pragma unroll
      for (int c = 0; c < CH; ++c) x[u][c] = stream_load(p + voff[c]);
      sbv[u] = a.sb[rc];
    }
    __builtin_amdgcn_sched_barrier(0);
#pragma unroll
    for (int u = 0; u < UR; ++u) {
      int a0 = 0, a1 = 0, a2 = 0;
#pragma unroll
      for (int c = 0; c < CH; ++c) {
        const unsigned xs[4] = {x[u][c].x, x[u][c].y, x[u][c].z, x[u][c].w};
#pragma unroll
        for (int k = 0; k < 4; ++k) {
          const int cw = (int)(xs[k] ^ 0x88888888u);
          a0 = __builtin_amdgcn_sdot8(cw, qp[c][k][0], a0, false);
          a1 = __builtin_amdgcn_sdot8(cw, qp[c][k][1], a1, false);
          a2 = __builtin_amdgcn_sdot8(cw, qp[c][k][2], a2, false);
        }
      }
      const int tot = group_allsum_i32<G>((a2 * 16 + a1) * 16 + a0);
      const float s4 = (sbv[u].x * h.qstep) * (float)tot;
      const float e4 = fmaf(sbv[u].y, h.eA, h.eB) + fabsf(s4) * 5e-7f;
      const float U4 = s4 + e4;
      const int64_t rw = r0 + (int64_t)(u * WAVES + wave) * RPW + rsub;
      const bool want = rw < n && sub == 0 && !(U4 < h.Lg);
      const unsigned long long bal = __ballot(want);
      if (bal) {
        const int pos = cnt + (int)__builtin_amdgcn_mbcnt_hi((unsigned)(bal >> 32), __builtin_amdgcn_mbcnt_lo((unsigned)bal, 0u));
        if (want && pos < a.seg_cap) seg[pos] = (int)rw;
        cnt += __popcll(bal);
      }
    }
  }
  if (lane == 0) a.counts[b] = cnt;
}

struct Second8Args {
  const uint4* Aq;
  const float2* sb;
  const float* q;
  const DevState* st;
  const int* list;
  const int* counts;
  PartialView out;
  int ldv, d, seg_cap;
  float kacc, err_coef;
};

template <int G, int CH, int UR>
__global__ __launch_bounds__(BCX_SCAN_THREADS) void second8_kernel(Second8Args a) {
  if (!a.st->active) return;
  constexpr int RPW = 64 / G;
  constexpr int WAVES = BCX_SCREEN_WAVES;
  const int lane = threadIdx.x & 63, wave = threadIdx.x >> 6;
  const int sub = lane % G, rsub = lane / G;
  const int b = blockIdx.x * WAVES + wave;
  const int cnt = __builtin_amdgcn_readfirstlane(a.counts[b]);
  const bool ovf = cnt > a.seg_cap;

  Track<float> tr;
  tr.U1 = tr.U2 = tr.U3 = tr.L = -INFINITY;
  tr.i1 = tr.i2 = 0x7fffffff;
  if (!ovf && cnt > 0) {
    Q16 q0[CH];
    int voff[CH];
    float qs0 = 0.0f;
#pragma unroll
    for (int c = 0; c < CH; ++c) {
      const int v = c * G + sub;
      const bool ok = v < a.ldv;
      voff[c] = ok ? v : 0;
      q0[c] = load_q16(a.q, v, a.d, ok, qs0);
    }
    const float off0 = -128.0f * qs0;
    const float qscale = (float)a.st->qscale;
    const int* seg = a.list + (size_t)b * BCX_S4_SEG_CAP;
    int nxt[UR];
#pragma unroll
    for (int u = 0; u < UR; ++u) { const int kk = u * RPW + rsub; nxt[u] = kk < cnt ? seg[kk] : -1; }
    for (int k0 = 0; k0 < cnt; k0 += RPW * UR) {
      int row[UR];
      uint4 x[UR][CH];
      float2 sbv[UR];
#pragma unroll
      for (int u = 0; u < UR; ++u) row[u] = nxt[u];
#pragma unroll
      for (int u = 0; u < UR; ++u) { const int kk = k0 + RPW * UR + u * RPW + rsub; nxt[u] = kk < cnt ? seg[kk] : -1; }
#pragma unroll
      for (int u = 0; u < UR; ++u) {
        const int64_t rc = row[u] < 0 ? 0 : row[u];
        const uint4* p = a.Aq + rc * a.ldv;
#pragma unroll
        for (int c = 0; c < CH; ++c) x[u][c] = stream_load(p + voff[c]);
        sbv[u] = a.sb[rc];
      }
      __builtin_amdgcn_sched_barrier(0);
#pragma unroll
      for (int u = 0; u < UR; ++u) {
        float t0 = off0;
#pragma unroll
        for (int c = 0; c < CH; ++c) t0 = dot16(x[u][c], q0[c], t0);
        float s0 = group_allsum<float, G>(t0);
        s0 *= sbv[u].x;
        float U, L;
        screen_interval(s0, sbv[u].x, sbv[u].y, a.kacc, a.err_coef, qscale, U, L);
        if (row[u] < 0) { U = -INFINITY; L = -INFINITY; }
        track_update<float>(tr, U, L, row[u] < 0 ? 0x7fffffff : row[u]);
      }
    }
#pragma unroll
    for (int off = G; off < 64; off <<= 1) tr = merge<float>(tr, shfl_track<float>(tr, off));
  }
  if (lane == 0) {
    if (ovf) {
      tr.U1 = tr.U2 = tr.L = -INFINITY; tr.U3 = INFINITY; tr.i1 = tr.i2 = 0x7fffffff;
    }
    a.out.U1[b] = (double)tr.U1; a.out.U2[b] = (double)tr.U2; a.out.U3[b] = (double)tr.U3; a.out.L[b] = (double)tr.L;
    a.out.i1[b] = tr.i1; a.out.i2[b] = tr.i2;
  }
}

template <bool F16>
__global__ __launch_bounds__(256) void quantise4_kernel(const void* An, int ld, int d, int nw4, int64_t n, unsigned* A4, float2* sb) {
  const int lane = threadIdx.x & 63;
  const int64_t row = (int64_t)blockIdx.x * 4 + (threadIdx.x >> 6);
  if (row >= n) return;
  auto elem = [&](int j) -> float {
    if (F16) return __half2float(((const __half*)An)[row * (int64_t)ld + j]);
    return ((const float*)An)[row * (int64_t)ld + j];
  };
  float m = 0.0f;
  for (int j = lane; j < d; j += 64) m = fmaxf(m, fabsf(elem(j)));
  m = (float)wave_allmax((double)m);
  float sc = (float)((double)m * BCX_S4_CLIP / 7.0);
  if (!(sc >= FLT_MIN)) sc = FLT_MIN;
  const double dsc = (double)sc;
  double r2 = 0.0;
  for (int w = lane; w < nw4; w += 64) {
    unsigned word = 0;
#pragma unroll
    for (int k = 0; k < 8; ++k) {
      const int j = 8 * w + k;
      int code = 0;
      if (j < d) {
        const double v = (double)elem(j);
        double c = rint(v / dsc);
        c = c > 7.0 ? 7.0 : (c < -7.0 ? -7.0 : c);
        if (c != c) c = 0.0;
        code = (int)c;
        const double r = v - c * dsc;
        r2 = fma(r, r, r2);
      }
      word |= (unsigned)(code + 8) << (4 * k);
    }
    A4[row * (int64_t)nw4 + w] = word;
  }
  r2 = wave_allsum(r2);
  if (lane == 0) {
    const double b = sqrt(r2) * (1.0 + 9.5367431640625e-07);
    float bf = (float)b;
    if ((double)bf < b) bf = nextafterf(bf, INFINITY);
    if (!(bf == bf)) bf = INFINITY;
    sb[row] = make_float2(sc, bf);
  }
}

bool bcx_screen4_on(const bcx_solver* s) {
  return s->s4_enabled && !s->s4_dropped && bcx_screen_on(s) && s->cfg.alg != BCX_ALG_GIGA && s->cfg.world_size == 1;
}

static size_t head_bytes(int nw4) { return sizeof(Front4Head) + (size_t)3 * nw4 * 4; }

int bcx_screen4_build(bcx_solver* s) {
  if (s->s4_valid || !bcx_screen4_on(s) || !s->scr_valid) return BCX_OK;
  const int d = s->cfg.d;
  const int64_t n = s->cfg.n_local;
  s->ld4 = (d + 31) / 32 * 16;
  const int nw4 = s->ld4 / 4;
  if (s->s4_cap_rows < n || !s->A4) {
    void** all[] = {&s->A4, &s->s4_sb, &s->s4_list, &s->s4_counts, &s->s4_head};
    for (void** p : all) { if (*p) (void)hipFree(*p); *p = nullptr; }
    s->s4_cap_rows = 0;
    hipError_t e = hipMalloc(&s->A4, (size_t)n * s->ld4);
    if (e == hipSuccess) e = hipMalloc(&s->s4_sb, (size_t)n * 8);
    if (e == hipSuccess) e = hipMalloc(&s->s4_list, (size_t)BCX_MAX_PARTIALS * BCX_S4_SEG_CAP * 4);
    if (e == hipSuccess) e = hipMalloc(&s->s4_counts, (size_t)BCX_MAX_PARTIALS * 4);
    if (e == hipSuccess) e = hipMalloc(&s->s4_head, head_bytes(nw4));
    if (e != hipSuccess) {
      (void)hipGetLastError();
      for (void** p : all) { if (*p) (void)hipFree(*p); *p = nullptr; }
      s->s4_dropped = 2;
      return BCX_OK;
    }
    s->s4_cap_rows = n;
    BCX_HIP(hipMemsetAsync(s->s4_counts, 0, (size_t)BCX_MAX_PARTIALS * 4, s->stream));
    BCX_HIP(hipMemsetAsync(s->scr_stat + SCR4_PENDING, 0, sizeof(unsigned long long), s->stream));
    s->s4_n_seg = 0;
  }
  const unsigned grid = (unsigned)((n + 3) / 4);
  if (s->cfg.store_dtype == BCX_F16)
    hipLaunchKernelGGL((quantise4_kernel<true>), dim3(grid), dim3(256), 0, s->stream, s->An, s->ld, d, nw4, n, (unsigned*)s->A4, (float2*)s->s4_sb);
  else
    hipLaunchKernelGGL((quantise4_kernel<false>), dim3(grid), dim3(256), 0, s->stream, s->An, s->ld, d, nw4, n, (unsigned*)s->A4, (float2*)s->s4_sb);
  BCX_HIP(hipGetLastError());
  s->s4_valid = true;
  s->s4_warm = 2;
  return BCX_OK;
}

static int launch_front4(bcx_solver* s, const Front4Args& a, int G, int CH, int UR, int grid) {
  dim3 g(grid), b(BCX_SCAN_THREADS);
#define L(GG, CC, UU)                                                                  \
  if (G == GG && CH == CC && UR == UU) {                                               \
    hipLaunchKernelGGL((front4_kernel<GG, CC, UU>), g, b, 0, s->stream, a);            \
    return BCX_OK;                                                                     \
  }
  L(1, 1, 4) L(2, 1, 4) L(4, 1, 4) L(8, 1, 4) L(16, 1, 4) L(32, 1, 4) L(64, 1, 4) L(64, 2, 4)
  L(1, 1, 8) L(2, 1, 8) L(4, 1, 8) L(8, 1, 8) L(16, 1, 8) L(32, 1, 8) L(64, 1, 8)
#undef L
  s->err = "front4: unsupported row length";
  return BCX_ERR_ARG;
}

static int launch_second8(bcx_solver* s, const Second8Args& a, int G, int CH, int grid) {
  dim3 g(grid), b(BCX_SCAN_THREADS);
#define L(GG, CC, UU)                                                                  \
  if (G == GG && CH == CC) {                                                           \
    hipLaunchKernelGGL((second8_kernel<GG, CC, UU>), g, b, 0, s->stream, a);           \
    return BCX_OK;                                                                     \
  }
  L(1, 1, 16) L(2, 1, 16) L(4, 1, 16) L(8, 1, 16) L(16, 1, 16) L(32, 1, 16) L(64, 1, 16) L(64, 2, 8) L(64, 4, 4)
#undef L
  s->err = "second8: unsupported row length";
  return BCX_ERR_ARG;
}

int bcx_launch_screen4(bcx_solver* s) {
  const int d = s->cfg.d;
  const int64_t n = s->cfg.n_local;
  const int nw4 = s->ld4 / 4;
  ScanArgs sa;
  ScanPlan sp;
  int rc = bcx_scan_plan(s, 0, &sa, &sp);
  if (rc != BCX_OK) return rc;
  const int ldv8 = s->ld8 / 16;
  const int G8 = screen_group(ldv8), CH8 = screen_chunks(ldv8, G8);
  const float kacc = screen_kacc(G8, CH8, d);

  Thresh4Args t;
  t.in = partial_view(s->scr_partials, s->scr_n_in); t.n_in = s->scr_n_in;
  t.Aq = (const unsigned char*)s->Aq; t.sb = (const float2*)s->scr_sb; t.q = (const float*)s->qst;
  t.st = s->st; t.stat = s->scr_stat; t.head = (unsigned*)s->s4_head;
  t.n = n; t.ld8 = s->ld8; t.d = d; t.nw4 = nw4;
  t.kacc = kacc; t.err_coef = sa.err_coef;

  Front4Args f;
  f.A4 = (const uint4*)s->A4; f.sb = (const float2*)s->s4_sb; f.head = (const unsigned*)s->s4_head; f.st = s->st;
  f.list = (int*)s->s4_list; f.counts = (int*)s->s4_counts;
  f.n = n; f.ldv = s->ld4 / 16; f.nw4 = nw4;
  const int G = screen_group(f.ldv), CH = screen_chunks(f.ldv, G);
  const int ur = CH == 1 ? 8 : 4;
  const int rpb = BCX_SCREEN_WAVES * (64 / G) * ur;
  const int64_t want = (n + rpb - 1) / rpb;
  int cap = 512;
  if (cap > BCX_MAX_PARTIALS / BCX_SCREEN_WAVES) cap = BCX_MAX_PARTIALS / BCX_SCREEN_WAVES;
  const int grid = (int)(want < 1 ? 1 : (want > cap ? cap : want));
  t.counts = (const int*)s->s4_counts; t.n_seg = s->s4_n_seg; t.seg_cap = s->s4_seg_cap;
  f.seg_cap = s->s4_seg_cap;
  hipLaunchKernelGGL(thresh4_kernel, dim3(1), dim3(BCX_THRESH_THREADS), 0, s->stream, t);
  BCX_HIP(hipGetLastError());
  s->s4_n_seg = grid * BCX_SCREEN_WAVES;
  if ((rc = launch_front4(s, f, G, CH, ur, grid))) return rc;

  const int n_in = grid * BCX_SCREEN_WAVES;
  Second8Args c;
  c.Aq = (const uint4*)s->Aq; c.sb = (const float2*)s->scr_sb; c.q = (const float*)s->qst; c.st = s->st;
  c.list = (const int*)s->s4_list; c.counts = (const int*)s->s4_counts;
  c.out = partial_view(s->scr_partials, n_in);
  c.ldv = ldv8; c.d = d; c.seg_cap = s->s4_seg_cap; c.kacc = kacc; c.err_coef = sa.err_coef;
  if ((rc = launch_second8(s, c, G8, CH8, grid))) return rc;
  BCX_HIP(hipGetLastError());
  s->scr_n_in = n_in;
  return bcx_launch_refine(s, n_in);
}
```

bayesian-coresets_amd/csrc/screen8.hip:

```cpp
#include <float.h>
#include "screen_core.h"

#define BCX_REFINE_THREADS 1024

struct ScreenArgs {
  const uint4* Aq;
  const float2* sb;
  const float* q;
  const DevState* st;
  PartialView out;
  int64_t n;
  int ldv;
  int ldq;
  int d;
  float kacc;
  float err_coef;
};

template <bool DUAL, int G, int CH, int UR>
__global__ __launch_bounds__(BCX_SCAN_THREADS) void screen_kernel(ScreenArgs a) {
  if (!a.st->active) return;
  constexpr int RPW = 64 / G;
  constexpr int WAVES = BCX_SCREEN_WAVES;
  constexpr int RPB = WAVES * RPW * UR;
  constexpr bool PACK4 = G >= 4 && (UR % 4 == 0);
  constexpr int GSZ = PACK4 ? G / 4 : G;
  constexpr int NT = PACK4 ? UR / 4 : UR;
  const int lane = threadIdx.x & 63, wave = threadIdx.x >> 6;
  const int sub = lane % G, rsub = lane / G;
  int myu = 0, myrs = 0;
  if constexpr (PACK4) pack_map<G>(lane, myu, myrs);

  Q16 q0[CH], q1[CH];
  int voff[CH];
  float qs0 = 0.0f, qs1 = 0.0f;
#pragma unroll
  for (int c = 0; c < CH; ++c) {
    const int v = c * G + sub;
    const bool ok = v < a.ldv;
    voff[c] = ok ? v : 0;
    q0[c] = load_q16(a.q, v, a.d, ok, qs0);
    if (DUAL) q1[c] = load_q16(a.q + a.ldq, v, a.d, ok, qs1);
  }
  const float off0 = -128.0f * qs0, off1 = -128.0f * qs1;
  const float qscale = (float)a.st->qscale;

  Track<float> tr;
  tr.U1 = tr.U2 = tr.U3 = tr.L = -INFINITY;
  tr.i1 = tr.i2 = 0x7fffffff;

  const uint4* base = a.Aq;
  const int64_t n = a.n;
  auto row_of = [&](int64_t r0, int u) { return r0 + (int64_t)(u * WAVES + wave) * RPW + rsub; };
  auto tracked = [&](int64_t r0, int t) {
    if constexpr (PACK4) return r0 + (int64_t)((t * 4 + myu) * WAVES + wave) * RPW + myrs;
    else return row_of(r0, t);
  };
  const int64_t stride = (int64_t)gridDim.x * RPB;
  for (int64_t r0 = (int64_t)blockIdx.x * RPB; r0 < n; r0 += stride) {
    uint4 x[UR][CH];
    float2 sbv[NT];
#pragma unroll
    for (int u = 0; u < UR; ++u) {
      const int64_t rw = row_of(r0, u);
      const int64_t rc = rw < n ? rw : n - 1;
      const uint4* p = base + rc * a.ldv;
#pragma unroll
      for (int c = 0; c < CH; ++c) x[u][c] = stream_load(p + voff[c]);
    }
#pragma unroll
    for (int t = 0; t < NT; ++t) { const int64_t rw = tracked(r0, t); sbv[t] = a.sb[rw < n ? rw : n - 1]; }
    __builtin_amdgcn_sched_barrier(0);
#pragma unroll
    for (int t = 0; t < NT; ++t) {
      float s0, s1 = 0.0f;
      if constexpr (PACK4) {
        float a0[4], a1[4];
#pragma unroll
        for (int u = 0; u < 4; ++u) {
          float t0 = off0, t1 = off1;
#pragma unroll
          for (int c = 0; c < CH; ++c) {
            t0 = dot16(x[t * 4 + u][c], q0[c], t0);
            if (DUAL) t1 = dot16(x[t * 4 + u][c], q1[c], t1);
          }
          a0[u] = t0; a1[u] = t1;
        }
        s0 = reduce4_pack<G, float>(a0[0], a0[1], a0[2], a0[3]);
        if (DUAL) s1 = reduce4_pack<G, float>(a1[0], a1[1], a1[2], a1[3]);
      } else {
        float t0 = off0, t1 = off1;
#pragma unroll
        for (int c = 0; c < CH; ++c) {
          t0 = dot16(x[t][c], q0[c], t0);
          if (DUAL) t1 = dot16(x[t][c], q1[c], t1);
        }
        s0 = group_allsum<float, G>(t0);
        if (DUAL) s1 = group_allsum<float, G>(t1);
      }
      const int64_t myrow = tracked(r0, t);
      const float scale = sbv[t].x, bound = sbv[t].y;
      s0 *= scale; s1 *= scale;
      float U, L;
      if (DUAL) giga_interval(s0, s1, (fmaf(scale, a.kacc, bound) * 1.000002f + a.err_coef) * qscale, U, L);
      else screen_interval(s0, scale, bound, a.kacc, a.err_coef, qscale, U, L);
      if (!(myrow < n)) { U = -INFINITY; L = -INFINITY; }
      track_update<float>(tr, U, L, (int)myrow);
    }
  }
#pragma unroll
  for (int off = GSZ; off < 64; off <<= 1) tr = merge<float>(tr, shfl_track<float>(tr, off));
  if (lane == 0) {
    const int b = blockIdx.x * WAVES + wave;
    a.out.U1[b] = (double)tr.U1; a.out.U2[b] = (double)tr.U2; a.out.U3[b] = (double)tr.U3; a.out.L[b] = (double)tr.L;
    a.out.i1[b] = tr.i1; a.out.i2[b] = tr.i2;
  }
}

struct RefineArgs {
  PartialView in;
  int n_in;
  PartialView out;
  DevState* st;
  unsigned long long* stat;
  const void* An;
  const float* q;
  int store_f16, ld, ldq, d, dual;
  double coef_mid;
};

__global__ __launch_bounds__(BCX_REFINE_THREADS) void refine_kernel(RefineArgs a) {
  if (!a.st->active) return;
  __shared__ double scratch[BCX_SCRATCH];
  __shared__ int surv[BCX_SCREEN_MAX_SURV];
  __shared__ int nsurv, overflow;
  constexpr int PP = BCX_MAX_PARTIALS / BCX_REFINE_THREADS;
  const int tid = threadIdx.x, lane = tid & 63, wave = tid >> 6, nwaves = BCX_REFINE_THREADS / 64;
  double u1[PP], u2[PP], u3[PP], lo[PP];
  int r1[PP], r2[PP];
#pragma unroll
  for (int t = 0; t < PP; ++t) {
    const int p = tid + t * BCX_REFINE_THREADS;
    const bool ok = p < a.n_in;
    u1[t] = ok ? a.in.U1[p] : -INFINITY; u2[t] = ok ? a.in.U2[p] : -INFINITY;
    u3[t] = ok ? a.in.U3[p] : -INFINITY; lo[t] = ok ? a.in.L[p] : -INFINITY;
    r1[t] = ok ? a.in.i1[p] : 0; r2[t] = ok ? a.in.i2[p] : 0;
  }
  if (tid == 0) { nsurv = 0; overflow = 0; }
  double lmax = -INFINITY;
#pragma unroll
  for (int t = 0; t < PP; ++t) lmax = fmax(lmax, lo[t]);
  const double Lstar = block_allmax(lmax, scratch);
#pragma unroll
  for (int t = 0; t < PP; ++t) {
    if (u1[t] > -INFINITY && u1[t] >= Lstar) { const int s = atomicAdd(&nsurv, 1); if (s < BCX_SCREEN_MAX_SURV) surv[s] = r1[t]; }
    if (u2[t] > -INFINITY && u2[t] >= Lstar) { const int s = atomicAdd(&nsurv, 1); if (s < BCX_SCREEN_MAX_SURV) surv[s] = r2[t]; }
    if (u3[t] > -INFINITY && u3[t] >= Lstar) overflow = 1;
  }
  __syncthreads();
  const int ns = nsurv;
  const bool ovf = overflow || ns > BCX_SCREEN_MAX_SURV;
  for (int p = tid; p < BCX_SCREEN_MAX_SURV; p += BCX_REFINE_THREADS) {
    if (ovf || p >= ns) {
      const bool mark = ovf && p == 0;
      a.out.U1[p] = -INFINITY; a.out.U2[p] = -INFINITY; a.out.U3[p] = mark ? INFINITY : -INFINITY; a.out.L[p] = mark ? 0.0 : -INFINITY;
      a.out.i1[p] = 0x7fffffff; a.out.i2[p] = 0x7fffffff;
    }
  }
  if (tid == 0) {
    a.stat[SCR_ARMED] = 1ull;
    atomicAdd(&a.stat[SCR_ITERS], 1ull);
    if (ovf) atomicAdd(&a.stat[SCR_OVERFLOWS], 1ull); else atomicAdd(&a.stat[SCR_SURVIVORS], (unsigned long long)ns);
  }
  if (ovf) return;
  const double qs = a.st->qscale;
  const double e = a.coef_mid * qs;
  for (int c = wave; c < ns; c += nwaves) {
    const int64_t i = surv[c];
    double s0 = 0.0, s1 = 0.0;
    for (int j = lane; j < a.d; j += 64) {
      const double v = a.store_f16 ? (double)__half2float(((const __half*)a.An)[i * (int64_t)a.ld + j])
                                   : (double)((const float*)a.An)[i * (int64_t)a.ld + j];
      s0 = fma(v, (double)a.q[j], s0);
      if (a.dual) s1 = fma(v, (double)a.q[a.ldq + j], s1);
    }
    s0 = wave_allsum(s0);
    if (a.dual) s1 = wave_allsum(s1);
    if (lane == 0) {
      double U, L;
      if (a.dual) {
        float Uf, Lf;
        giga_interval((float)s0, (float)s1, (float)(e * 1.000001) , Uf, Lf);
        U = Uf; L = Lf;
      } else { U = s0 + e; L = s0 - e; }
      a.out.U1[c] = U; a.out.L[c] = L; a.out.i1[c] = (int)i;
      a.out.U2[c] = -INFINITY; a.out.U3[c] = -INFINITY; a.out.i2[c] = 0x7fffffff;
    }
  }
}

__global__ __launch_bounds__(64) void resume_store_kernel(DevState* st, unsigned long long* stat) {
  if (threadIdx.x == 0 && st->halt == HALT_NEED_EXACT && stat[SCR_ARMED]) {
    st->active = 1; st->halt = HALT_NONE; st->exact_mode = 0;
    stat[SCR_ARMED] = 0ull; stat[SCR_REDOS] += 1ull;
  }
}

template <bool F16>
__global__ __launch_bounds__(256) void quantise_kernel(const void* An, int ld, int d, int ld8, int64_t n, unsigned* Aq, float2* sb) {
  const int lane = threadIdx.x & 63;
  const int64_t row = (int64_t)blockIdx.x * 4 + (threadIdx.x >> 6);
  if (row >= n) return;
  auto elem = [&](int j) -> float {
    if (F16) return __half2float(((const __half*)An)[row * (int64_t)ld + j]);
    return ((const float*)An)[row * (int64_t)ld + j];
  };
  float m = 0.0f;
  for (int j = lane; j < d; j += 64) m = fmaxf(m, fabsf(elem(j)));
  m = (float)wave_allmax((double)m);
  float sc = (float)((double)m / 127.0);
  if (!(sc >= FLT_MIN)) sc = FLT_MIN;
  const double dsc = (double)sc;
  double r2 = 0.0;
  const int nw = ld8 / 4;
  for (int w = lane; w < nw; w += 64) {
    unsigned word = 0;
#pragma unroll
    for (int k = 0; k < 4; ++k) {
      const int j = 4 * w + k;
      int code = 0;
      if (j < d) {
        const double v = (double)elem(j);
        double c = rint(v / dsc);
        c = c > 127.0 ? 127.0 : (c < -127.0 ? -127.0 : c);
        if (c != c) c = 0.0;
        code = (int)c;
        const double r = v - c * dsc;
        r2 = fma(r, r, r2);
      }
      word |= (unsigned)(code + 128) << (8 * k);
    }
    Aq[row * (int64_t)nw + w] = word;
  }
  r2 = wave_allsum(r2);
  if (lane == 0) {
    const double b = sqrt(r2) * (1.0 + 9.5367431640625e-07);
    float bf = (float)b;
    if ((double)bf < b) bf = nextafterf(bf, INFINITY);
    if (!(bf == bf)) bf = INFINITY;
    sb[row] = make_float2(sc, bf);
  }
}

static bool screen_applicable(const bcx_solver* s) {
  return s->cfg.store_dtype != BCX_F64 && s->cfg.d <= 64 * 4 * 16 && s->cfg.n_local > 0;
}

bool bcx_screen_on(const bcx_solver* s) { return s->scr_enabled && !s->scr_dropped && screen_applicable(s); }

int bcx_screen_build(bcx_solver* s) {
  if (s->scr_valid || !bcx_screen_on(s)) return BCX_OK;
  const int d = s->cfg.d;
  const int64_t n = s->cfg.n_local;
  s->ld8 = (d + 15) / 16 * 16;
  const size_t need = (size_t)n * s->ld8;
  hipError_t e = hipSuccess;
  if (s->scr_cap_rows < n || !s->Aq) {
    if (s->Aq) (void)hipFree(s->Aq);
    if (s->scr_sb) (void)hipFree(s->scr_sb);
    s->Aq = nullptr; s->scr_sb = nullptr; s->scr_cap_rows = 0;
    e = hipMalloc(&s->Aq, need);
    if (e == hipSuccess) e = hipMalloc(&s->scr_sb, (size_t)n * 8);
    if (e == hipSuccess && !s->scr_partials) e = hipMalloc(&s->scr_partials, (size_t)BCX_MAX_PARTIALS * BCX_PARTIAL_BYTES);
    if (e == hipSuccess && !s->scr_stat) {
      e = hipMalloc((void**)&s->scr_stat, SCR_WORDS * sizeof(unsigned long long));
      if (e == hipSuccess) e = hipMemset(s->scr_stat, 0, SCR_WORDS * sizeof(unsigned long long));
    }
    if (e != hipSuccess) {
      (void)hipGetLastError();
      if (s->Aq) (void)hipFree(s->Aq);
      if (s->scr_sb) (void)hipFree(s->scr_sb);
      s->Aq = nullptr; s->scr_sb = nullptr;
      s->scr_dropped = 2;
      return BCX_OK;
    }
    s->scr_cap_rows = n;
  }
  hipEvent_t e0, e1;
  BCX_HIP(hipEventCreate(&e0));
  BCX_HIP(hipEventCreate(&e1));
  BCX_HIP(hipEventRecord(e0, s->stream));
  const unsigned grid = (unsigned)((n + 3) / 4);
  if (s->cfg.store_dtype == BCX_F16)
    hipLaunchKernelGGL((quantise_kernel<true>), dim3(grid), dim3(256), 0, s->stream, s->An, s->ld, d, s->ld8, n, (unsigned*)s->Aq, (float2*)s->scr_sb);
  else
    hipLaunchKernelGGL((quantise_kernel<false>), dim3(grid), dim3(256), 0, s->stream, s->An, s->ld, d, s->ld8, n, (unsigned*)s->Aq, (float2*)s->scr_sb);
  BCX_HIP(hipGetLastError());
  BCX_HIP(hipEventRecord(e1, s->stream));
  BCX_HIP(hipEventSynchronize(e1));
  float ms = 0.f;
  BCX_HIP(hipEventElapsedTime(&ms, e0, e1));
  (void)hipEventDestroy(e0); (void)hipEventDestroy(e1);
  s->scr_build_ms = ms;
  s->scr_valid = true;
  return BCX_OK;
}

template <bool DUAL> static int launch_screen_t(bcx_solver* s, const ScreenArgs& a, int G, int CH, int UR, int grid) {
  dim3 g(grid), b(BCX_SCAN_THREADS);
#define L(GG, CC, UU)                                                                            \
  if (G == GG && CH == CC && UR == UU) {                                                         \
    hipLaunchKernelGGL((screen_kernel<DUAL, GG, CC, UU>), g, b, 0, s->stream, a);                \
    return BCX_OK;                                                                               \
  }
  L(1, 1, 4) L(2, 1, 4) L(4, 1, 4) L(8, 1, 4) L(16, 1, 4) L(32, 1, 4) L(64, 1, 4) L(64, 2, 4) L(64, 4, 4)
  L(4, 1, 8) L(8, 1, 8) L(16, 1, 8) L(32, 1, 8) L(64, 1, 8)
#undef L
  s->err = "screen: unsupported row length";
  return BCX_ERR_ARG;
}

int bcx_launch_screen(bcx_solver* s) {
  const int d = s->cfg.d;
  ScreenArgs a;
  a.Aq = (const uint4*)s->Aq;
  a.sb = (const float2*)s->scr_sb;
  a.q = (const float*)s->qst;
  a.ldq = s->ld;
  a.st = s->st;
  a.n = s->cfg.n_local;
  a.ldv = s->ld8 / 16;
  a.d = d;
  const int G = screen_group(a.ldv);
  const int CH = screen_chunks(a.ldv, G);
  a.kacc = screen_kacc(G, CH, d);
  ScanArgs sa;
  ScanPlan sp;
  int rc = bcx_scan_plan(s, 0, &sa, &sp);
  if (rc != BCX_OK) return rc;
  a.err_coef = sa.err_coef;
  int ur = 4;
  if (const char* e = bcx_dev_env("BCX_SCREEN_UR")) { if (atoi(e) == 8 && CH == 1 && G >= 4) ur = 8; }
  const int rpb = BCX_SCREEN_WAVES * (64 / G) * ur;
  int64_t want = (a.n + rpb - 1) / rpb;
  int cap = (CH * ur >= 8) ? 256 : 512;
  if (const char* e = bcx_dev_env("BCX_SCREEN_GRID")) { const long v = atol(e); if (v > 0) cap = (int)v; }
  if (cap > BCX_MAX_PARTIALS / BCX_SCREEN_WAVES) cap = BCX_MAX_PARTIALS / BCX_SCREEN_WAVES;
  const int grid = (int)(want < 1 ? 1 : (want > cap ? cap : want));
  const int n_in = grid * BCX_SCREEN_WAVES;
  a.out = partial_view(s->scr_partials, n_in);
  const bool dual = s->cfg.alg == BCX_ALG_GIGA;
  rc = dual ? launch_screen_t<true>(s, a, G, CH, ur, grid) : launch_screen_t<false>(s, a, G, CH, ur, grid);
  if (rc != BCX_OK) return rc;
  s->scr_n_in = n_in;
  return bcx_launch_refine(s, n_in);
}

int bcx_launch_refine(bcx_solver* s, int n_in) {
  const int d = s->cfg.d;
  const bool f16 = s->cfg.store_dtype == BCX_F16;
  const double u = 5.9604644775390625e-08;
  RefineArgs r;
  r.in = partial_view(s->scr_partials, n_in); r.n_in = n_in;
  r.out = partial_view(s->partials, BCX_SCREEN_MAX_SURV);
  r.st = s->st; r.stat = s->scr_stat;
  r.An = s->An; r.q = (const float*)s->qst;
  r.store_f16 = f16; r.ld = s->ld; r.ldq = s->ld; r.d = d; r.dual = s->cfg.alg == BCX_ALG_GIGA;
  r.coef_mid = 1.3 * u * 3.0;
  if (f16) r.coef_mid += 1.02 * (4.8828125e-4 + 2.9802322387695312e-08 * sqrt((double)d));
  hipLaunchKernelGGL(refine_kernel, dim3(1), dim3(BCX_REFINE_THREADS), 0, s->stream, r);
  BCX_HIP(hipGetLastError());
  s->n_partials = BCX_SCREEN_MAX_SURV;
  return BCX_OK;
}

int bcx_launch_resume_store(bcx_solver* s) {
  hipLaunchKernelGGL(resume_store_kernel, dim3(1), dim3(64), 0, s->stream, s->st, s->scr_stat);
  BCX_HIP(hipGetLastError());
  return BCX_OK;
}
```

Baseline: 2249.

## Fuse 4-bit screen threshold and 8-bit settle into front4 kernel

Removes the single-block thresh4 kernel and the separate second8 kernel. Sentinel row selection moves into the refine kernel, which writes a sentinel list for the next iteration. Each front4 block now recomputes the threshold head (sentinel dot products and query plane packing) redundantly in shared memory, overlapped with its first row loads, and settles its own segment list at 8 bits inline. The refine kernel also prefetches the first survivor row and takes over the listed/overflow statistics. This cuts per-iteration launches and serial single-block work at the cost of redundant per-block head computation, and it uses sentinels taken from the previous iteration.

```diff
diff --git a/bayesian-coresets_amd/csrc/api.hip b/bayesian-coresets_amd/csrc/api.hip
--- a/bayesian-coresets_amd/csrc/api.hip
+++ b/bayesian-coresets_amd/csrc/api.hip
@@ -36,7 +36,7 @@
   for (size_t w = 0; w < s->peer_mbox.size(); ++w)
     if (s->peer_mbox[w] && s->peer_mbox[w] != s->mbox) (void)hipIpcCloseMemHandle(s->peer_mbox[w]);
   void* xptrs[] = {s->mbox, s->peer_tab, s->xseq, s->xprobe, s->rec_gather, s->grid_counter, s->fin_part, s->gram_work, s->warm_buf,
-                   s->Aq, s->scr_sb, s->scr_partials, s->scr_stat, s->A4, s->s4_sb, s->s4_list, s->s4_counts, s->s4_head};
+                   s->Aq, s->scr_sb, s->scr_partials, s->scr_stat, s->A4, s->s4_sb, s->s4_list, s->s4_counts, s->s4_sent};
   for (void* p : xptrs)
     if (p) (void)hipFree(p);
   for (auto& ev : s->prof_events) { (void)hipEventDestroy(ev.first); (void)hipEventDestroy(ev.second); }
@@ -630,7 +630,7 @@
     unsigned long long st8[SCR_WORDS];
     BCX_HIP(hipMemcpy(st8, s->scr_stat, sizeof st8, hipMemcpyDeviceToHost));
     if (!st8[SCR_ARMED]) break;
-    if (st8[SCR4_LAST] != 0 && st8[SCR4_LAST] == st8[SCR_ITERS]) {
+    if (st8[SCR4_LAST] != 0) {
       s->s4_halts += 1;
       for (int i = 3; i > 0; --i) s->s4_ovf_at[i] = s->s4_ovf_at[i - 1];
       s->s4_ovf_at[0] = st8[SCR4_ITERS];
@@ -944,11 +944,6 @@
   }
   const bool possible = s->s4_enabled && s->scr_enabled && s->cfg.store_dtype != BCX_F64 && s->cfg.d <= 4096 && s->cfg.n_local > 0 &&
                         s->cfg.alg != BCX_ALG_GIGA && s->cfg.world_size == 1;
-  if (st8[SCR4_PENDING] && s->s4_counts && s->s4_n_seg > 0) {
-    std::vector<int32_t> cnt((size_t)s->s4_n_seg);
-    BCX_HIP(hipMemcpy(cnt.data(), s->s4_counts, cnt.size() * 4, hipMemcpyDeviceToHost));
-    for (int32_t c : cnt) { st8[SCR4_LISTED] += (unsigned long long)std::min<int32_t>(c, s->s4_seg_cap); st8[SCR4_OVERFLOWS] += c > s->s4_seg_cap; }
-  }
   out8[0] = bcx_screen4_on(s) ? 1 : 0;
   out8[1] = (int64_t)st8[SCR4_ITERS];
   out8[2] = (int64_t)st8[SCR4_LISTED];
diff --git a/bayesian-coresets_amd/csrc/bcx_internal.h b/bayesian-coresets_amd/csrc/bcx_internal.h
--- a/bayesian-coresets_amd/csrc/bcx_internal.h
+++ b/bayesian-coresets_amd/csrc/bcx_internal.h
@@ -35,8 +35,7 @@
        SCR4_LISTED = 6,
        SCR4_OVERFLOWS = 7,
        SCR4_LAST = 8,
-       SCR4_PENDING = 9,
-       SCR_WORDS = 10 };
+       SCR_WORDS = 9 };
 #define BCX_S4_SEG_CAP 1024
 #define BCX_S4_SENTINELS 64
 static inline __host__ __device__ PartialView partial_view(void* base, int n) {
@@ -183,9 +182,8 @@
   void* s4_sb = nullptr;
   void* s4_list = nullptr;
   void* s4_counts = nullptr;
-  void* s4_head = nullptr;
+  void* s4_sent = nullptr;
   int ld4 = 0;
-  int s4_n_seg = 0;
   int s4_seg_cap = BCX_S4_SEG_CAP;
   int64_t s4_cap_rows = 0;
   bool s4_enabled = true;
@@ -229,7 +227,7 @@
 int bcx_screen_build(bcx_solver* s);
 int bcx_launch_screen(bcx_solver* s);
 int bcx_launch_resume_store(bcx_solver* s);
-int bcx_launch_refine(bcx_solver* s, int n_in);
+int bcx_launch_refine(bcx_solver* s, int n_in, bool four);
 bool bcx_screen4_on(const bcx_solver* s);
 int bcx_screen4_build(bcx_solver* s);
 int bcx_launch_screen4(bcx_solver* s);
diff --git a/bayesian-coresets_amd/csrc/screen4.hip b/bayesian-coresets_amd/csrc/screen4.hip
--- a/bayesian-coresets_amd/csrc/screen4.hip
+++ b/bayesian-coresets_amd/csrc/screen4.hip
@@ -3,7 +3,7 @@
 
 #define BCX_S4_CLIP 0.8
 #define BCX_S4_QMAX 1911.0
-#define BCX_THRESH_THREADS 1024
+#define BCX_S4_MAX_NW4 512
 
 struct Front4Head { float Lg, qstep, eA, eB; };
 
@@ -24,103 +24,102 @@
   return f;
 }
 
-struct Thresh4Args {
-  PartialView in;
-  int n_in;
-  const unsigned char* Aq;
+struct Front4Args {
+  const uint4* A4;
   const float2* sb;
   const float* q;
+  const int* sent;
+  const unsigned char* Aq;
+  const float2* sb8;
   const DevState* st;
-  unsigned long long* stat;
-  unsigned* head;
-  const int* counts;
-  int n_seg;
-  int seg_cap;
+  int* list;
+  int* counts;
   int64_t n;
-  int ld8, d, nw4;
+  int ldv, nw4, seg_cap;
+  int ld8, d;
   float kacc, err_coef;
+  PartialView out;
+  int ldv8;
 };
 
-__global__ __launch_bounds__(BCX_THRESH_THREADS) void thresh4_kernel(Thresh4Args a) {
-  if (!a.st->active) return;
-  __shared__ double scratch[BCX_SCRATCH];
+#define BCX_S4_SPW (BCX_S4_SENTINELS / BCX_SCREEN_WAVES)
+
+static __device__ __forceinline__ Front4Head front4_head(const Front4Args& a, int myrow, float2 mysb, float qscale,
+                                                         unsigned* planes, double* scratch) {
   const int tid = threadIdx.x, lane = tid & 63, wave = tid >> 6;
-  constexpr int NW = BCX_THRESH_THREADS / 64;
-  constexpr int PT = 2 * BCX_MAX_PARTIALS / BCX_THRESH_THREADS;
-  double cu[PT];
-  int ci[PT];
-#pragma unroll
-  for (int t = 0; t < PT; ++t) {
-    const int c = wave + NW * (lane + 64 * t);
-    const int p = c >> 1;
-    const bool ok = p < a.n_in;
-    const double u = ok ? ((c & 1) ? a.in.U2[p] : a.in.U1[p]) : -INFINITY;
-    const int i = ok ? ((c & 1) ? a.in.i2[p] : a.in.i1[p]) : -1;
-    const bool use = u > -INFINITY && i >= 0 && (int64_t)i < a.n;
-    cu[t] = use ? u : -INFINITY; ci[t] = use ? i : -1;
-  }
+  constexpr int NW = BCX_SCREEN_WAVES;
+  constexpr int SPW = BCX_S4_SPW;
+  int rows[SPW];
+#pragma unroll
+  for (int r = 0; r < SPW; ++r) rows[r] = __builtin_amdgcn_readlane(myrow, r);
+  double acc[SPW];
+#pragma unroll
+  for (int r = 0; r < SPW; ++r) acc[r] = 0.0;
   double m = 0.0;
-  for (int j = tid; j < a.d; j += BCX_THRESH_THREADS) {
-    const double v = fabs((double)a.q[j]);
-    m = fmax(m, v == v ? v : INFINITY);
-  }
-  m = block_allmax(m, scratch);
+  const int nw8 = a.ld8 / 4;
+  const unsigned* A8 = (const unsigned*)a.Aq;
+  for (int w0 = lane; w0 < nw8; w0 += 128) {
+    unsigned cw[2][SPW];
+    float qf[2][4];
+#pragma unroll
+    for (int h = 0; h < 2; ++h) {
+      const int w = w0 + 64 * h;
+      const int wc = w < nw8 ? w : 0;
+#pragma unroll
+      for (int k = 0; k < 4; ++k) { const int j = 4 * w + k; qf[h][k] = a.q[(w < nw8 && j < a.d) ? j : 0]; }
+#pragma unroll
+      for (int r = 0; r < SPW; ++r) cw[h][r] = A8[(int64_t)(rows[r] < 0 ? 0 : rows[r]) * nw8 + wc];
+    }
+    __builtin_amdgcn_sched_barrier(0);
+    double qv[2][4];
+#pragma unroll
+    for (int h = 0; h < 2; ++h)
+#pragma unroll
+      for (int k = 0; k < 4; ++k) {
+        const int w = w0 + 64 * h, j = 4 * w + k;
+        qv[h][k] = (w < nw8 && j < a.d) ? (double)qf[h][k] : 0.0;
+        const double v = fabs(qv[h][k]);
+        m = fmax(m, v == v ? v : INFINITY);
+      }
+#pragma unroll
+    for (int h = 0; h < 2; ++h)
+#pragma unroll
+      for (int r = 0; r < SPW; ++r)
+#pragma unroll
+        for (int k = 0; k < 4; ++k) acc[r] = fma((double)((int)((cw[h][r] >> (8 * k)) & 0xffu) - 128), qv[h][k], acc[r]);
+  }
+  double tot = 0.0;
+#pragma unroll
+  for (int r = 0; r < SPW; ++r) { const double t = wave_allsum(acc[r]); tot = (lane & (SPW - 1)) == r ? t : tot; }
+  float lmax = -INFINITY;
+  {
+    const float s0 = (float)((double)mysb.x * tot);
+    float U, L;
+    screen_interval(s0, mysb.x, mysb.y, a.kacc, a.err_coef, qscale, U, L);
+    if (myrow >= 0) lmax = fmaxf(lmax, L);
+  }
+  lmax = (float)wave_allmax((double)lmax);
+  m = wave_allmax(m);
   float step = (float)(m / BCX_S4_QMAX);
   const bool qok = m < INFINITY && step >= FLT_MIN;
   if (!qok) step = 0.0f;
-  constexpr int SPW = BCX_S4_SENTINELS / NW;
-  int rows[SPW];
-#pragma unroll
-  for (int r = 0; r < SPW; ++r) {
-    double best = -INFINITY;
-    int bt = -1, bi = -1;
-#pragma unroll
-    for (int t = 0; t < PT; ++t) if (cu[t] > best) { best = cu[t]; bt = t; bi = ci[t]; }
-    const double wm = wave_allmax(best);
-    const unsigned long long bal = __ballot(bt >= 0 && best == wm);
-    const int src = bal ? __ffsll((long long)bal) - 1 : 0;
-    const int row = __shfl(bi, src, BCX_WAVE);
-    rows[r] = bal ? row : -1;
-#pragma unroll
-    for (int t = 0; t < PT; ++t) if (bal && lane == src && t == bt) cu[t] = -INFINITY;
-  }
-  double acc[SPW];
-#pragma unroll
-  for (int r = 0; r < SPW; ++r) acc[r] = 0.0;
-  const int nw8 = a.ld8 / 4;
-  const unsigned* A8 = (const unsigned*)a.Aq;
-  for (int w = lane; w < nw8; w += 64) {
-    unsigned cw[SPW];
-#pragma unroll
-    for (int r = 0; r < SPW; ++r) cw[r] = A8[(int64_t)(rows[r] < 0 ? 0 : rows[r]) * nw8 + w];
-    double qv[4];
-#pragma unroll
-    for (int k = 0; k < 4; ++k) { const int j = 4 * w + k; const float t = a.q[j < a.d ? j : 0]; qv[k] = j < a.d ? (double)t : 0.0; }
-#pragma unroll
-    for (int r = 0; r < SPW; ++r)
-#pragma unroll
-      for (int k = 0; k < 4; ++k) acc[r] = fma((double)((int)((cw[r] >> (8 * k)) & 0xffu) - 128), qv[k], acc[r]);
-  }
-  double err2[3] = {0.0, 0.0, 0.0};
-  if (a.stat[SCR4_PENDING])
-    for (int p = tid; p < a.n_seg; p += BCX_THRESH_THREADS) {
-      const int c = a.counts[p];
-      err2[1] += (double)(c > a.seg_cap ? a.seg_cap : c);
-      err2[2] += c > a.seg_cap ? 1.0 : 0.0;
-    }
-  for (int w = tid; w < a.nw4; w += BCX_THRESH_THREADS) {
+  double err2 = 0.0;
+  for (int w = tid; w < a.nw4; w += BCX_SCAN_THREADS) {
     unsigned p0 = 0, p1 = 0, p2 = 0;
+    float q8[8];
+#pragma unroll
+    for (int k = 0; k < 8; ++k) { const int j = 8 * w + k; q8[k] = a.q[j < a.d ? j : 0]; }
 #pragma unroll
     for (int k = 0; k < 8; ++k) {
       const int j = 8 * w + k;
       int x = 0;
       if (j < a.d && qok) {
-        const double v = (double)a.q[j];
+        const double v = (double)q8[k];
         double c = rint(v / (double)step);
         c = c > BCX_S4_QMAX ? BCX_S4_QMAX : (c < -BCX_S4_QMAX ? -BCX_S4_QMAX : c);
         x = (int)c;
         const double r = v - c * (double)step;
-        err2[0] = fma(r, r, err2[0]);
+        err2 = fma(r, r, err2);
       }
       const int l = ((x + 8) & 15) - 8;
       const int x1 = (x - l) >> 4;
@@ -128,82 +127,125 @@
       const int h2 = (x1 - h1) >> 4;
       p0 |= (unsigned)(l & 15) << (4 * k); p1 |= (unsigned)(h1 & 15) << (4 * k); p2 |= (unsigned)(h2 & 15) << (4 * k);
     }
-    a.head[4 + w] = p0; a.head[4 + a.nw4 + w] = p1; a.head[4 + 2 * a.nw4 + w] = p2;
-  }
-  block_allsum<3>(err2, scratch);
-  const double qerr = sqrt(err2[0]) * (1.0 + 9.5367431640625e-07);
+    planes[w] = p0; planes[a.nw4 + w] = p1; planes[2 * a.nw4 + w] = p2;
+  }
+  err2 = wave_allsum(err2);
+  if (lane == 0) { scratch[wave] = err2; scratch[NW + wave] = (double)lmax; }
+  __syncthreads();
+  err2 = scratch[0];
+  double lg = scratch[NW];
+#pragma unroll
+  for (int w = 1; w < NW; ++w) { err2 += scratch[w]; lg = fmax(lg, scratch[NW + w]); }
+  const double qerr = sqrt(err2) * (1.0 + 9.5367431640625e-07);
+  const double qs = (double)qscale;
+  Front4Head h;
+  h.Lg = qok ? (float)lg : -INFINITY;
+  h.qstep = step;
+  h.eA = round_up_f32((qs * 1.000002 + qerr) * 1.000004);
+  h.eB = round_up_f32(((double)a.err_coef * qs + 1.001 * qerr) * 1.000004 + 1e-37);
+  return h;
+}
+
+template <int G, int CH, int UR>
+__device__ __forceinline__ void settle8(const Front4Args& a, const int* seg, int b, int cnt, float qscale) {
+  constexpr int RPW = 64 / G;
+  const int lane = threadIdx.x & 63;
+  const int sub = lane % G, rsub = lane / G;
+  const bool ovf = cnt > a.seg_cap;
+
+  Track<float> tr;
+  tr.U1 = tr.U2 = tr.U3 = tr.L = -INFINITY;
+  tr.i1 = tr.i2 = 0x7fffffff;
+  if (!ovf && cnt > 0) {
+    Q16 q0[CH];
+    int voff[CH];
+    float qs0 = 0.0f;
+#pragma unroll
+    for (int c = 0; c < CH; ++c) {
+      const int v = c * G + sub;
+      const bool ok = v < a.ldv8;
+      voff[c] = ok ? v : 0;
+      q0[c] = load_q16(a.q, v, a.d, ok, qs0);
+    }
+    const float off0 = -128.0f * qs0;
+    int nxt[UR];
+#pragma unroll
+    for (int u = 0; u < UR; ++u) { const int kk = u * RPW + rsub; nxt[u] = kk < cnt ? seg[kk] : -1; }
+    for (int k0 = 0; k0 < cnt; k0 += RPW * UR) {
+      int row[UR];
+      uint4 x[UR][CH];
+      float2 sbv[UR];
+#pragma unroll
+      for (int u = 0; u < UR; ++u) row[u] = nxt[u];
+#pragma unroll
+      for (int u = 0; u < UR; ++u) { const int kk = k0 + RPW * UR + u * RPW + rsub; nxt[u] = kk < cnt ? seg[kk] : -1; }
+#pragma unroll
+      for (int u = 0; u < UR; ++u) {
+        const int64_t rc = row[u] < 0 ? 0 : row[u];
+        const uint4* p = (const uint4*)a.Aq + rc * a.ldv8;
+#pragma unroll
+        for (int c = 0; c < CH; ++c) x[u][c] = stream_load(p + voff[c]);
+        sbv[u] = a.sb8[rc];
+      }
+      __builtin_amdgcn_sched_barrier(0);
+#pragma unroll
+      for (int u = 0; u < UR; ++u) {
+        float t0 = off0;
+#pragma unroll
+        for (int c = 0; c < CH; ++c) t0 = dot16(x[u][c], q0[c], t0);
+        float s0 = group_allsum<float, G>(t0);
+        s0 *= sbv[u].x;
+        float U, L;
+        screen_interval(s0, sbv[u].x, sbv[u].y, a.kacc, a.err_coef, qscale, U, L);
+        if (row[u] < 0) { U = -INFINITY; L = -INFINITY; }
+        track_update<float>(tr, U, L, row[u] < 0 ? 0x7fffffff : row[u]);
+      }
+    }
+#pragma unroll
+    for (int off = G; off < 64; off <<= 1) tr = merge<float>(tr, shfl_track<float>(tr, off));
+  }
+  if (lane == 0) {
+    if (ovf) {
+      tr.U1 = tr.U2 = tr.L = -INFINITY; tr.U3 = INFINITY; tr.i1 = tr.i2 = 0x7fffffff;
+    }
+    a.out.U1[b] = (double)tr.U1; a.out.U2[b] = (double)tr.U2; a.out.U3[b] = (double)tr.U3; a.out.L[b] = (double)tr.L;
+    a.out.i1[b] = tr.i1; a.out.i2[b] = tr.i2;
+  }
+}
+
+template <int G, int CH, int UR, int G8, int CH8, int UR8>
+__global__ __launch_bounds__(BCX_SCAN_THREADS) void front4_kernel(Front4Args a) {
+  int myrow = a.sent[(threadIdx.x >> 6) * BCX_S4_SPW + (threadIdx.x & (BCX_S4_SPW - 1))];
   const float qscale = (float)a.st->qscale;
-  float lmax = -INFINITY;
-#pragma unroll
-  for (int r = 0; r < SPW; ++r) {
-    const double tot = wave_allsum(acc[r]);
-    const float2 sb = a.sb[rows[r] < 0 ? 0 : rows[r]];
-    const float s0 = (float)((double)sb.x * tot);
-    float U, L;
-    screen_interval(s0, sb.x, sb.y, a.kacc, a.err_coef, qscale, U, L);
-    if (rows[r] >= 0) lmax = fmaxf(lmax, L);
-  }
-  const double lg = block_allmax((double)lmax, scratch);
-  if (tid == 0) {
-    const double qs = (double)qscale;
-    Front4Head h;
-    h.Lg = qok ? (float)lg : -INFINITY;
-    h.qstep = step;
-    h.eA = round_up_f32((qs * 1.000002 + qerr) * 1.000004);
-    h.eB = round_up_f32(((double)a.err_coef * qs + 1.001 * qerr) * 1.000004 + 1e-37);
-    *(Front4Head*)a.head = h;
-    a.stat[SCR4_LAST] = a.stat[SCR_ITERS] + 1ull;
-    a.stat[SCR4_ITERS] += 1ull;
-    a.stat[SCR4_LISTED] += (unsigned long long)err2[1];
-    a.stat[SCR4_OVERFLOWS] += (unsigned long long)err2[2];
-    a.stat[SCR4_PENDING] = 1ull;
-  }
-}
-
-struct Front4Args {
-  const uint4* A4;
-  const float2* sb;
-  const unsigned* head;
-  const DevState* st;
-  int* list;
-  int* counts;
-  int64_t n;
-  int ldv, nw4, seg_cap;
-};
-
-template <int G, int CH, int UR>
-__global__ __launch_bounds__(BCX_SCAN_THREADS) void front4_kernel(Front4Args a) {
-  if (!a.st->active) return;
+  const int active = a.st->active;
+  asm volatile("" : "+v"(myrow));
+  if (!active) return;
+  if (!(myrow >= 0 && (int64_t)myrow < a.n)) myrow = -1;
+  const float2 mysb = a.sb8[myrow < 0 ? 0 : myrow];
+  __shared__ double scratch[BCX_SCRATCH];
+  __shared__ unsigned planes[3 * BCX_S4_MAX_NW4];
+  __shared__ int lseg[BCX_SCREEN_WAVES][BCX_S4_SEG_CAP];
   constexpr int RPW = 64 / G;
   constexpr int WAVES = BCX_SCREEN_WAVES;
   constexpr int RPB = WAVES * RPW * UR;
   const int lane = threadIdx.x & 63, wave = threadIdx.x >> 6;
   const int sub = lane % G, rsub = lane / G;
-  const Front4Head h = *(const Front4Head*)a.head;
-  const unsigned* planes = a.head + 4;
-  int qp[CH][4][3];
   int voff[CH];
+  bool vok[CH];
 #pragma unroll
   for (int c = 0; c < CH; ++c) {
     const int v = c * G + sub;
-    const bool ok = v < a.ldv;
-    voff[c] = ok ? v : 0;
-#pragma unroll
-    for (int k = 0; k < 4; ++k)
-#pragma unroll
-      for (int p = 0; p < 3; ++p) {
-        const unsigned w = planes[p * a.nw4 + 4 * voff[c] + k];
-        qp[c][k][p] = ok ? (int)w : 0;
-      }
+    vok[c] = v < a.ldv;
+    voff[c] = vok[c] ? v : 0;
   }
   const int b = blockIdx.x * WAVES + wave;
   int* seg = a.list + (size_t)b * BCX_S4_SEG_CAP;
   int cnt = 0;
   const int64_t n = a.n;
   const int64_t stride = (int64_t)gridDim.x * RPB;
-  for (int64_t r0 = (int64_t)blockIdx.x * RPB; r0 < n; r0 += stride) {
-    uint4 x[UR][CH];
-    float2 sbv[UR];
+  uint4 x[UR][CH];
+  float2 sbv[UR];
+  auto load_trip = [&](int64_t r0) {
 #pragma unroll
     for (int u = 0; u < UR; ++u) {
       const int64_t rw = r0 + (int64_t)(u * WAVES + wave) * RPW + rsub;
@@ -213,6 +255,19 @@
       for (int c = 0; c < CH; ++c) x[u][c] = stream_load(p + voff[c]);
       sbv[u] = a.sb[rc];
     }
+  };
+  int64_t r0 = (int64_t)blockIdx.x * RPB;
+  load_trip(r0);
+  __builtin_amdgcn_sched_barrier(0);
+  const Front4Head h = front4_head(a, myrow, mysb, qscale, planes, scratch);
+  int qp[CH][4][3];
+#pragma unroll
+  for (int c = 0; c < CH; ++c)
+#pragma unroll
+    for (int k = 0; k < 4; ++k)
+#pragma unroll
+      for (int p = 0; p < 3; ++p) qp[c][k][p] = vok[c] ? (int)planes[p * a.nw4 + 4 * voff[c] + k] : 0;
+  for (;;) {
     __builtin_amdgcn_sched_barrier(0);
 #pragma unroll
     for (int u = 0; u < UR; ++u) {
@@ -237,97 +292,16 @@
       const unsigned long long bal = __ballot(want);
       if (bal) {
         const int pos = cnt + (int)__builtin_amdgcn_mbcnt_hi((unsigned)(bal >> 32), __builtin_amdgcn_mbcnt_lo((unsigned)bal, 0u));
-        if (want && pos < a.seg_cap) seg[pos] = (int)rw;
+        if (want && pos < a.seg_cap) { seg[pos] = (int)rw; lseg[wave][pos] = (int)rw; }
         cnt += __popcll(bal);
       }
     }
+    r0 += stride;
+    if (!(r0 < n)) break;
+    load_trip(r0);
   }
   if (lane == 0) a.counts[b] = cnt;
-}
-
-struct Second8Args {
-  const uint4* Aq;
-  const float2* sb;
-  const float* q;
-  const DevState* st;
-  const int* list;
-  const int* counts;
-  PartialView out;
-  int ldv, d, seg_cap;
-  float kacc, err_coef;
-};
-
-template <int G, int CH, int UR>
-__global__ __launch_bounds__(BCX_SCAN_THREADS) void second8_kernel(Second8Args a) {
-  if (!a.st->active) return;
-  constexpr int RPW = 64 / G;
-  constexpr int WAVES = BCX_SCREEN_WAVES;
-  const int lane = threadIdx.x & 63, wave = threadIdx.x >> 6;
-  const int sub = lane % G, rsub = lane / G;
-  const int b = blockIdx.x * WAVES + wave;
-  const int cnt = __builtin_amdgcn_readfirstlane(a.counts[b]);
-  const bool ovf = cnt > a.seg_cap;
-
-  Track<float> tr;
-  tr.U1 = tr.U2 = tr.U3 = tr.L = -INFINITY;
-  tr.i1 = tr.i2 = 0x7fffffff;
-  if (!ovf && cnt > 0) {
-    Q16 q0[CH];
-    int voff[CH];
-    float qs0 = 0.0f;
-#pragma unroll
-    for (int c = 0; c < CH; ++c) {
-      const int v = c * G + sub;
-      const bool ok = v < a.ldv;
-      voff[c] = ok ? v : 0;
-      q0[c] = load_q16(a.q, v, a.d, ok, qs0);
-    }
-    const float off0 = -128.0f * qs0;
-    const float qscale = (float)a.st->qscale;
-    const int* seg = a.list + (size_t)b * BCX_S4_SEG_CAP;
-    int nxt[UR];
-#pragma unroll
-    for (int u = 0; u < UR; ++u) { const int kk = u * RPW + rsub; nxt[u] = kk < cnt ? seg[kk] : -1; }
-    for (int k0 = 0; k0 < cnt; k0 += RPW * UR) {
-      int row[UR];
-      uint4 x[UR][CH];
-      float2 sbv[UR];
-#pragma unroll
-      for (int u = 0; u < UR; ++u) row[u] = nxt[u];
-#pragma unroll
-      for (int u = 0; u < UR; ++u) { const int kk = k0 + RPW * UR + u * RPW + rsub; nxt[u] = kk < cnt ? seg[kk] : -1; }
-#pragma unroll
-      for (int u = 0; u < UR; ++u) {
-        const int64_t rc = row[u] < 0 ? 0 : row[u];
-        const uint4* p = a.Aq + rc * a.ldv;
-#pragma unroll
-        for (int c = 0; c < CH; ++c) x[u][c] = stream_load(p + voff[c]);
-        sbv[u] = a.sb[rc];
-      }
-      __builtin_amdgcn_sched_barrier(0);
-#pragma unroll
-      for (int u = 0; u < UR; ++u) {
-        float t0 = off0;
-#pragma unroll
-        for (int c = 0; c < CH; ++c) t0 = dot16(x[u][c], q0[c], t0);
-        float s0 = group_allsum<float, G>(t0);
-        s0 *= sbv[u].x;
-        float U, L;
-        screen_interval(s0, sbv[u].x, sbv[u].y, a.kacc, a.err_coef, qscale, U, L);
-        if (row[u] < 0) { U = -INFINITY; L = -INFINITY; }
-        track_update<float>(tr, U, L, row[u] < 0 ? 0x7fffffff : row[u]);
-      }
-    }
-#pragma unroll
-    for (int off = G; off < 64; off <<= 1) tr = merge<float>(tr, shfl_track<float>(tr, off));
-  }
-  if (lane == 0) {
-    if (ovf) {
-      tr.U1 = tr.U2 = tr.L = -INFINITY; tr.U3 = INFINITY; tr.i1 = tr.i2 = 0x7fffffff;
-    }
-    a.out.U1[b] = (double)tr.U1; a.out.U2[b] = (double)tr.U2; a.out.U3[b] = (double)tr.U3; a.out.L[b] = (double)tr.L;
-    a.out.i1[b] = tr.i1; a.out.i2[b] = tr.i2;
-  }
+  settle8<G8, CH8, UR8>(a, lseg[wave], b, cnt, qscale);
 }
 
 template <bool F16>
@@ -379,8 +353,6 @@
   return s->s4_enabled && !s->s4_dropped && bcx_screen_on(s) && s->cfg.alg != BCX_ALG_GIGA && s->cfg.world_size == 1;
 }
 
-static size_t head_bytes(int nw4) { return sizeof(Front4Head) + (size_t)3 * nw4 * 4; }
-
 int bcx_screen4_build(bcx_solver* s) {
   if (s->s4_valid || !bcx_screen4_on(s) || !s->scr_valid) return BCX_OK;
   const int d = s->cfg.d;
@@ -388,14 +360,14 @@
   s->ld4 = (d + 31) / 32 * 16;
   const int nw4 = s->ld4 / 4;
   if (s->s4_cap_rows < n || !s->A4) {
-    void** all[] = {&s->A4, &s->s4_sb, &s->s4_list, &s->s4_counts, &s->s4_head};
+    void** all[] = {&s->A4, &s->s4_sb, &s->s4_list, &s->s4_counts, &s->s4_sent};
     for (void** p : all) { if (*p) (void)hipFree(*p); *p = nullptr; }
     s->s4_cap_rows = 0;
     hipError_t e = hipMalloc(&s->A4, (size_t)n * s->ld4);
     if (e == hipSuccess) e = hipMalloc(&s->s4_sb, (size_t)n * 8);
     if (e == hipSuccess) e = hipMalloc(&s->s4_list, (size_t)BCX_MAX_PARTIALS * BCX_S4_SEG_CAP * 4);
     if (e == hipSuccess) e = hipMalloc(&s->s4_counts, (size_t)BCX_MAX_PARTIALS * 4);
-    if (e == hipSuccess) e = hipMalloc(&s->s4_head, head_bytes(nw4));
+    if (e == hipSuccess) e = hipMalloc(&s->s4_sent, (size_t)BCX_S4_SENTINELS * 4);
     if (e != hipSuccess) {
       (void)hipGetLastError();
       for (void** p : all) { if (*p) (void)hipFree(*p); *p = nullptr; }
@@ -403,9 +375,7 @@
       return BCX_OK;
     }
     s->s4_cap_rows = n;
-    BCX_HIP(hipMemsetAsync(s->s4_counts, 0, (size_t)BCX_MAX_PARTIALS * 4, s->stream));
-    BCX_HIP(hipMemsetAsync(s->scr_stat + SCR4_PENDING, 0, sizeof(unsigned long long), s->stream));
-    s->s4_n_seg = 0;
+    BCX_HIP(hipMemsetAsync(s->s4_sent, 0xff, (size_t)BCX_S4_SENTINELS * 4, s->stream));
   }
   const unsigned grid = (unsigned)((n + 3) / 4);
   if (s->cfg.store_dtype == BCX_F16)
@@ -418,30 +388,17 @@
   return BCX_OK;
 }
 
-static int launch_front4(bcx_solver* s, const Front4Args& a, int G, int CH, int UR, int grid) {
+static int launch_front4(bcx_solver* s, const Front4Args& a, int G, int CH, int G8, int CH8, int grid) {
   dim3 g(grid), b(BCX_SCAN_THREADS);
-#define L(GG, CC, UU)                                                                  \
-  if (G == GG && CH == CC && UR == UU) {                                               \
-    hipLaunchKernelGGL((front4_kernel<GG, CC, UU>), g, b, 0, s->stream, a);            \
-    return BCX_OK;                                                                     \
-  }
-  L(1, 1, 4) L(2, 1, 4) L(4, 1, 4) L(8, 1, 4) L(16, 1, 4) L(32, 1, 4) L(64, 1, 4) L(64, 2, 4)
-  L(1, 1, 8) L(2, 1, 8) L(4, 1, 8) L(8, 1, 8) L(16, 1, 8) L(32, 1, 8) L(64, 1, 8)
+#define L(GG, CC, UU, G8_, C8_, U8_)                                                                   \
+  if (G == GG && CH == CC && G8 == G8_ && CH8 == C8_) {                                                \
+    hipLaunchKernelGGL((front4_kernel<GG, CC, UU, G8_, C8_, U8_>), g, b, 0, s->stream, a);             \
+    return BCX_OK;                                                                                     \
+  }
+  L(1, 1, 8, 1, 1, 16) L(1, 1, 8, 2, 1, 16) L(2, 1, 8, 4, 1, 16) L(4, 1, 8, 8, 1, 16) L(8, 1, 8, 16, 1, 16)
+  L(16, 1, 8, 32, 1, 16) L(32, 1, 8, 64, 1, 16) L(64, 1, 8, 64, 2, 8) L(64, 2, 4, 64, 4, 4)
 #undef L
   s->err = "front4: unsupported row length";
-  return BCX_ERR_ARG;
-}
-
-static int launch_second8(bcx_solver* s, const Second8Args& a, int G, int CH, int grid) {
-  dim3 g(grid), b(BCX_SCAN_THREADS);
-#define L(GG, CC, UU)                                                                  \
-  if (G == GG && CH == CC) {                                                           \
-    hipLaunchKernelGGL((second8_kernel<GG, CC, UU>), g, b, 0, s->stream, a);           \
-    return BCX_OK;                                                                     \
-  }
-  L(1, 1, 16) L(2, 1, 16) L(4, 1, 16) L(8, 1, 16) L(16, 1, 16) L(32, 1, 16) L(64, 1, 16) L(64, 2, 8) L(64, 4, 4)
-#undef L
-  s->err = "second8: unsupported row length";
   return BCX_ERR_ARG;
 }
 
@@ -449,6 +406,7 @@
   const int d = s->cfg.d;
   const int64_t n = s->cfg.n_local;
   const int nw4 = s->ld4 / 4;
+  if (nw4 > BCX_S4_MAX_NW4) { s->err = "front4: unsupported row length"; return BCX_ERR_ARG; }
   ScanArgs sa;
   ScanPlan sp;
   int rc = bcx_scan_plan(s, 0, &sa, &sp);
@@ -457,17 +415,12 @@
   const int G8 = screen_group(ldv8), CH8 = screen_chunks(ldv8, G8);
   const float kacc = screen_kacc(G8, CH8, d);
 
-  Thresh4Args t;
-  t.in = partial_view(s->scr_partials, s->scr_n_in); t.n_in = s->scr_n_in;
-  t.Aq = (const unsigned char*)s->Aq; t.sb = (const float2*)s->scr_sb; t.q = (const float*)s->qst;
-  t.st = s->st; t.stat = s->scr_stat; t.head = (unsigned*)s->s4_head;
-  t.n = n; t.ld8 = s->ld8; t.d = d; t.nw4 = nw4;
-  t.kacc = kacc; t.err_coef = sa.err_coef;
-
   Front4Args f;
-  f.A4 = (const uint4*)s->A4; f.sb = (const float2*)s->s4_sb; f.head = (const unsigned*)s->s4_head; f.st = s->st;
+  f.A4 = (const uint4*)s->A4; f.sb = (const float2*)s->s4_sb; f.q = (const float*)s->qst; f.sent = (const int*)s->s4_sent;
+  f.Aq = (const unsigned char*)s->Aq; f.sb8 = (const float2*)s->scr_sb; f.st = s->st;
   f.list = (int*)s->s4_list; f.counts = (int*)s->s4_counts;
-  f.n = n; f.ldv = s->ld4 / 16; f.nw4 = nw4;
+  f.n = n; f.ldv = s->ld4 / 16; f.nw4 = nw4; f.seg_cap = s->s4_seg_cap;
+  f.ld8 = s->ld8; f.d = d; f.kacc = kacc; f.err_coef = sa.err_coef;
   const int G = screen_group(f.ldv), CH = screen_chunks(f.ldv, G);
   const int ur = CH == 1 ? 8 : 4;
   const int rpb = BCX_SCREEN_WAVES * (64 / G) * ur;
@@ -475,21 +428,11 @@
   int cap = 512;
   if (cap > BCX_MAX_PARTIALS / BCX_SCREEN_WAVES) cap = BCX_MAX_PARTIALS / BCX_SCREEN_WAVES;
   const int grid = (int)(want < 1 ? 1 : (want > cap ? cap : want));
-  t.counts = (const int*)s->s4_counts; t.n_seg = s->s4_n_seg; t.seg_cap = s->s4_seg_cap;
-  f.seg_cap = s->s4_seg_cap;
-  hipLaunchKernelGGL(thresh4_kernel, dim3(1), dim3(BCX_THRESH_THREADS), 0, s->stream, t);
-  BCX_HIP(hipGetLastError());
-  s->s4_n_seg = grid * BCX_SCREEN_WAVES;
-  if ((rc = launch_front4(s, f, G, CH, ur, grid))) return rc;
 
   const int n_in = grid * BCX_SCREEN_WAVES;
-  Second8Args c;
-  c.Aq = (const uint4*)s->Aq; c.sb = (const float2*)s->scr_sb; c.q = (const float*)s->qst; c.st = s->st;
-  c.list = (const int*)s->s4_list; c.counts = (const int*)s->s4_counts;
-  c.out = partial_view(s->scr_partials, n_in);
-  c.ldv = ldv8; c.d = d; c.seg_cap = s->s4_seg_cap; c.kacc = kacc; c.err_coef = sa.err_coef;
-  if ((rc = launch_second8(s, c, G8, CH8, grid))) return rc;
+  f.out = partial_view(s->scr_partials, n_in); f.ldv8 = ldv8;
+  if ((rc = launch_front4(s, f, G, CH, G8, CH8, grid))) return rc;
   BCX_HIP(hipGetLastError());
   s->scr_n_in = n_in;
-  return bcx_launch_refine(s, n_in);
-}
+  return bcx_launch_refine(s, n_in, true);
+}
diff --git a/bayesian-coresets_amd/csrc/screen8.hip b/bayesian-coresets_amd/csrc/screen8.hip
--- a/bayesian-coresets_amd/csrc/screen8.hip
+++ b/bayesian-coresets_amd/csrc/screen8.hip
@@ -127,17 +127,23 @@
   const float* q;
   int store_f16, ld, ldq, d, dual;
   double coef_mid;
+  int* sent;
+  const int* counts;
+  int seg_cap;
+  int64_t n;
 };
+
+#define BCX_REFINE_PF 8
 
 __global__ __launch_bounds__(BCX_REFINE_THREADS) void refine_kernel(RefineArgs a) {
   if (!a.st->active) return;
   __shared__ double scratch[BCX_SCRATCH];
   __shared__ int surv[BCX_SCREEN_MAX_SURV];
-  __shared__ int nsurv, overflow;
+  __shared__ int nsurv, overflow, listed, full;
   constexpr int PP = BCX_MAX_PARTIALS / BCX_REFINE_THREADS;
   const int tid = threadIdx.x, lane = tid & 63, wave = tid >> 6, nwaves = BCX_REFINE_THREADS / 64;
   double u1[PP], u2[PP], u3[PP], lo[PP];
-  int r1[PP], r2[PP];
+  int r1[PP], r2[PP], cn[PP];
 #pragma unroll
   for (int t = 0; t < PP; ++t) {
     const int p = tid + t * BCX_REFINE_THREADS;
@@ -145,8 +151,9 @@
     u1[t] = ok ? a.in.U1[p] : -INFINITY; u2[t] = ok ? a.in.U2[p] : -INFINITY;
     u3[t] = ok ? a.in.U3[p] : -INFINITY; lo[t] = ok ? a.in.L[p] : -INFINITY;
     r1[t] = ok ? a.in.i1[p] : 0; r2[t] = ok ? a.in.i2[p] : 0;
-  }
-  if (tid == 0) { nsurv = 0; overflow = 0; }
+    cn[t] = (ok && a.counts) ? a.counts[p] : 0;
+  }
+  if (tid == 0) { nsurv = 0; overflow = 0; listed = 0; full = 0; }
   double lmax = -INFINITY;
 #pragma unroll
   for (int t = 0; t < PP; ++t) lmax = fmax(lmax, lo[t]);
@@ -156,6 +163,13 @@
     if (u1[t] > -INFINITY && u1[t] >= Lstar) { const int s = atomicAdd(&nsurv, 1); if (s < BCX_SCREEN_MAX_SURV) surv[s] = r1[t]; }
     if (u2[t] > -INFINITY && u2[t] >= Lstar) { const int s = atomicAdd(&nsurv, 1); if (s < BCX_SCREEN_MAX_SURV) surv[s] = r2[t]; }
     if (u3[t] > -INFINITY && u3[t] >= Lstar) overflow = 1;
+  }
+  if (a.counts) {
+    double li = 0.0, fu = 0.0;
+#pragma unroll
+    for (int t = 0; t < PP; ++t) { li += (double)(cn[t] > a.seg_cap ? a.seg_cap : cn[t]); fu += cn[t] > a.seg_cap ? 1.0 : 0.0; }
+    li = wave_allsum(li); fu = wave_allsum(fu);
+    if (lane == 0) { atomicAdd(&listed, (int)li); atomicAdd(&full, (int)fu); }
   }
   __syncthreads();
   const int ns = nsurv;
@@ -171,6 +185,56 @@
     a.stat[SCR_ARMED] = 1ull;
     atomicAdd(&a.stat[SCR_ITERS], 1ull);
     if (ovf) atomicAdd(&a.stat[SCR_OVERFLOWS], 1ull); else atomicAdd(&a.stat[SCR_SURVIVORS], (unsigned long long)ns);
+    a.stat[SCR4_LAST] = a.counts ? 1ull : 0ull;
+    if (a.counts) {
+      atomicAdd(&a.stat[SCR4_ITERS], 1ull);
+      atomicAdd(&a.stat[SCR4_LISTED], (unsigned long long)listed);
+      atomicAdd(&a.stat[SCR4_OVERFLOWS], (unsigned long long)full);
+    }
+  }
+  auto stored = [&](int64_t i, int j) -> double {
+    return a.store_f16 ? (double)__half2float(((const __half*)a.An)[i * (int64_t)a.ld + j])
+                       : (double)((const float*)a.An)[i * (int64_t)a.ld + j];
+  };
+  double pv[BCX_REFINE_PF];
+  float pq0[BCX_REFINE_PF];
+  const bool ahead = a.sent && !a.dual && !ovf && wave < ns;
+#pragma unroll
+  for (int k = 0; k < BCX_REFINE_PF; ++k) { pv[k] = 0.0; pq0[k] = 0.0f; }
+  if (ahead) {
+    const int64_t row0 = surv[wave];
+#pragma unroll
+    for (int k = 0; k < BCX_REFINE_PF; ++k) {
+      const int j = lane + 64 * k, jc = j < a.d ? j : 0;
+      pv[k] = stored(row0, jc); pq0[k] = a.q[jc];
+    }
+  }
+  __builtin_amdgcn_sched_barrier(0);
+  if (a.sent) {
+    constexpr int SPW = BCX_S4_SENTINELS / (BCX_REFINE_THREADS / 64);
+    double cu[2 * PP];
+    int ci[2 * PP];
+#pragma unroll
+    for (int t = 0; t < 2 * PP; ++t) {
+      const double u = (t & 1) ? u2[t >> 1] : u1[t >> 1];
+      const int i = (t & 1) ? r2[t >> 1] : r1[t >> 1];
+      const bool use = u > -INFINITY && u < INFINITY && i >= 0 && (int64_t)i < a.n;
+      cu[t] = use ? u : -INFINITY; ci[t] = use ? i : -1;
+    }
+#pragma unroll
+    for (int r = 0; r < SPW; ++r) {
+      double best = -INFINITY;
+      int bt = -1, bi = -1;
+#pragma unroll
+      for (int t = 0; t < 2 * PP; ++t) if (cu[t] > best) { best = cu[t]; bt = t; bi = ci[t]; }
+      const double wm = wave_allmax(best);
+      const unsigned long long bal = __ballot(bt >= 0 && best == wm);
+      const int src = bal ? __ffsll((long long)bal) - 1 : 0;
+      const int row = __shfl(bi, src, BCX_WAVE);
+      if (lane == 0) a.sent[wave * SPW + r] = bal ? row : -1;
+#pragma unroll
+      for (int t = 0; t < 2 * PP; ++t) if (bal && lane == src && t == bt) cu[t] = -INFINITY;
+    }
   }
   if (ovf) return;
   const double qs = a.st->qscale;
@@ -178,9 +242,16 @@
   for (int c = wave; c < ns; c += nwaves) {
     const int64_t i = surv[c];
     double s0 = 0.0, s1 = 0.0;
-    for (int j = lane; j < a.d; j += 64) {
-      const double v = a.store_f16 ? (double)__half2float(((const __half*)a.An)[i * (int64_t)a.ld + j])
-                                   : (double)((const float*)a.An)[i * (int64_t)a.ld + j];
+    int j = lane;
+    if (ahead && c == wave) {
+#pragma unroll
+      for (int k = 0; k < BCX_REFINE_PF; ++k, j += 64) {
+        const double t0 = fma(pv[k], (double)pq0[k], s0);
+        s0 = j < a.d ? t0 : s0;
+      }
+    }
+    for (; j < a.d; j += 64) {
+      const double v = stored(i, j);
       s0 = fma(v, (double)a.q[j], s0);
       if (a.dual) s1 = fma(v, (double)a.q[a.ldq + j], s1);
     }
@@ -353,10 +424,10 @@
   rc = dual ? launch_screen_t<true>(s, a, G, CH, ur, grid) : launch_screen_t<false>(s, a, G, CH, ur, grid);
   if (rc != BCX_OK) return rc;
   s->scr_n_in = n_in;
-  return bcx_launch_refine(s, n_in);
-}
-
-int bcx_launch_refine(bcx_solver* s, int n_in) {
+  return bcx_launch_refine(s, n_in, false);
+}
+
+int bcx_launch_refine(bcx_solver* s, int n_in, bool four) {
   const int d = s->cfg.d;
   const bool f16 = s->cfg.store_dtype == BCX_F16;
   const double u = 5.9604644775390625e-08;
@@ -366,6 +437,8 @@
   r.st = s->st; r.stat = s->scr_stat;
   r.An = s->An; r.q = (const float*)s->qst;
   r.store_f16 = f16; r.ld = s->ld; r.ldq = s->ld; r.d = d; r.dual = s->cfg.alg == BCX_ALG_GIGA;
+  r.sent = bcx_screen4_on(s) ? (int*)s->s4_sent : nullptr;
+  r.counts = four ? (const int*)s->s4_counts : nullptr; r.seg_cap = s->s4_seg_cap; r.n = s->cfg.n_local;
   r.coef_mid = 1.3 * u * 3.0;
   if (f16) r.coef_mid += 1.02 * (4.8828125e-4 + 2.9802322387695312e-08 * sqrt((double)d));
   hipLaunchKernelGGL(refine_kernel, dim3(1), dim3(BCX_REFINE_THREADS), 0, s->stream, r);
```

Result: faster. 2347, median of 6 (+4.4%).
